# cpuimage/minSDTF

Measured on AMD Instinct MI355X. Metric: 512x512 images/sec (whole node), SD1.5 25-step txt2img, higher is better.
Workload: dtype bf16; 1 GPU; SD1.5 512x512 25-step txt2img, CFG 7.5 + rescale 0.7, batch 1/GPU, UNet+VAE HIP path, random-init weights; global_batch=1, parallelism=batch-shard x1, hipgraph=True, cond_uncond=one fused batch

## Files before the change

### include/minsdtf_hip.h

```cpp
#ifndef MINSDTF_HIP_H
#define MINSDTF_HIP_H

#include <stdint.h>

#ifdef __cplusplus
extern "C" {
#endif

#define MSD_ABI_VERSION 12

#define MSD_OK 0
#define MSD_E_ARG (-1)
#define MSD_E_ALIGN (-2)
#define MSD_E_UNSUPPORTED (-3)
#define MSD_E_WORKSPACE (-4)

typedef void* msd_stream_t;

#if defined(__GNUC__) || defined(__clang__)
#define MSD_API __attribute__((visibility("default")))
#else
#define MSD_API
#endif

MSD_API int msd_abi_version(void);
MSD_API const char* msd_last_error(void);
MSD_API int msd_init(void);
MSD_API int msd_set_option(const char* key, int value);

#define MSD_ACT_NONE 0
#define MSD_ACT_SILU 1
#define MSD_ACT_GEGLU 2
#define MSD_ACT_QUICK_GELU 3

#define MSD_OUT_BF16 0
#define MSD_OUT_F32 1

typedef struct MsdConvGemm {
    const void* a0;
    const void* a1;
    const void* w;
    const float* bias;
    const float* rowvec;
    const int32_t* step_ptr;
    const void* residual;
    void* out;
    void* out1;
    void* out2;
    float* workspace;
    int64_t workspace_floats;
    int32_t batch, h_in, w_in, c0, c1;
    int32_t h_out, w_out;
    int32_t ksize;
    int32_t stride;
    int32_t pad;
    int32_t upsample;
    int32_t N;
    int32_t act;
    int32_t out_dtype;
    int32_t out_ld, res_ld;
    int32_t rv_step_stride, rv_batch_stride;
    int32_t split_mode;
    int32_t ns0, ns1, out1_ld, out2_ld;
    int32_t splitk;
    int32_t tile_n;
    int32_t tile_m;
    int32_t stages;
    const float* ln_in;
    const float* ln_colsum;
    float* ln_out;
    int32_t ln_in_slots;
    int32_t ln_out_slots;
    float ln_eps;
    const void* a2;
    const void* a3;
    int32_t c2, c3;
    int32_t w_layout;
} MsdConvGemm;

MSD_API int msd_conv_gemm_ln_slots(const MsdConvGemm* p);

MSD_API int msd_conv_gemm(const MsdConvGemm* p, msd_stream_t stream);

#define MSD_OUT_U8 2
typedef struct MsdConvDirect {
    const void* in;
    const float* w;
    const float* bias;
    const void* residual;
    void* out;
    int32_t batch, in_batch_mod, h_in, w_in, c_in;
    int32_t h_out, w_out, c_out;
    int32_t ksize, stride, pad;
    int32_t in_dtype;
    int32_t out_dtype;
    int32_t act;
    int32_t act_in;
    float in_scale;
} MsdConvDirect;

MSD_API int msd_conv_direct(const MsdConvDirect* p, msd_stream_t stream);

#define MSD_GN_SYNC_WORDS_PER_SAMPLE 16384
#define MSD_GN_MAX_CHUNKS 1024
typedef struct MsdGroupNorm {
    const void* x0;
    const void* x1;
    const float* gamma;
    const float* beta;
    float* stats;
    float* partials;
    int64_t partials_floats;
    void* out;
    int32_t batch, hw, c0, c1;
    int32_t silu;
    float eps;
    uint32_t* sync;
    int64_t sync_words;
} MsdGroupNorm;

MSD_API int msd_group_norm(const MsdGroupNorm* p, msd_stream_t stream);

MSD_API int msd_layer_norm(const void* x, const float* gamma, const float* beta, void* out, int32_t rows, int32_t c,
                   float eps, msd_stream_t stream);

typedef struct MsdAttention {
    const void* q;
    const void* k;
    const void* vt;
    void* out;
    int32_t batch, heads, head_dim;
    int32_t s, t;
    int32_t q_ld, k_ld, vt_ld, o_ld;
    float scale;
    int32_t causal;
    int32_t q_prescaled;
    float* workspace;
    int64_t workspace_floats;
} MsdAttention;

MSD_API int msd_attention(const MsdAttention* p, msd_stream_t stream);

typedef struct MsdCrossAttnQ {
    const void* x;
    const float* ln_in;
    const void* wq;
    const float* ln_colsum;
    const float* bias;
    const void* k;
    const void* vt;
    void* out;
    int32_t batch, heads, head_dim, s, t;
    int32_t k_ld, vt_ld, o_ld;
    int32_t ln_in_slots;
    float ln_eps;
    int32_t w_layout;
} MsdCrossAttnQ;

MSD_API int msd_cross_attention_q(const MsdCrossAttnQ* p, msd_stream_t stream);

MSD_API int msd_softmax_rows(const float* x, void* out, int64_t rows, int32_t cols, int32_t ld_in, int32_t ld_out, float scale,
                     msd_stream_t stream);

MSD_API int msd_embedding_sum(const int32_t* tokens, const int32_t* positions, const float* tok_table, const float* pos_table,
                      void* out, int32_t rows, int32_t dim, int32_t vocab, int32_t max_len, int32_t* status,
                      msd_stream_t stream);

MSD_API int msd_replicate(const void* src, void* dst, int64_t bytes, int32_t copies, msd_stream_t stream);

MSD_API int msd_memset_zero(void* ptr, int64_t bytes, msd_stream_t stream);

typedef struct MsdCfgStep {
    const float* eps;
    float* latent;
    const float* coef;
    int32_t* step_ptr;
    int32_t batch, n, num_steps;
    float guidance, guidance_rescale;
    int32_t advance;
    const float* inpaint_init;
    const float* inpaint_noise;
    const float* inpaint_mask;
    const float* step_noise;
    const float* noise_coef;
} MsdCfgStep;

MSD_API int msd_cfg_step(const MsdCfgStep* p, msd_stream_t stream);

typedef struct MsdSamplerStep {
    const float* eps;
    float* latent;
    const float* coef;
    int32_t* step_ptr;
    int32_t batch, n, num_steps;
    float guidance, guidance_rescale;
    int32_t advance;
    const float* inpaint_init;
    const float* inpaint_noise;
    const float* inpaint_mask;
    const float* step_noise;
    float* denoised_prev;
} MsdSamplerStep;

MSD_API int msd_sampler_step(const MsdSamplerStep* p, msd_stream_t stream);

typedef struct MsdLoraJob {
    const float* master;
    const float* up;
    const float* down;
    const float* rowscale;
    const float* colscale;
    const int32_t* rowmap;
    void* out;
    void* out_frag;
    float* colsum;
    int32_t n, k, rank, master_ld;
    int32_t layout, out_dtype, ld;
    int32_t out_rows, out_cols, row_off, col_off;
    int32_t first_block;
} MsdLoraJob;

typedef struct MsdLoraMerge {
    const MsdLoraJob* jobs;
    const MsdLoraJob* jobs_dev;
    int32_t num_jobs;
} MsdLoraMerge;

MSD_API int msd_lora_merge(const MsdLoraMerge* p, msd_stream_t stream);

typedef struct MsdResampleRow {
// ... 62 lines not shown
```

### minsdtf_amd/_lib.py

```python
from __future__ import annotations

import atexit
import ctypes as C
import os
import sys
import weakref

LIB_NAME = "libminsdtf_hip.so"
LIB_PATH = os.environ.get("MSD_HIP_LIB") or os.path.join(os.path.dirname(os.path.abspath(__file__)), LIB_NAME)
ABI_VERSION = 12

ACT_NONE, ACT_SILU, ACT_GEGLU, ACT_QUICK_GELU = 0, 1, 2, 3
OUT_BF16, OUT_F32, OUT_U8 = 0, 1, 2


class HipExtensionError(RuntimeError):
    pass


class MsdConvGemm(C.Structure):
    _fields_ = [
        ("a0", C.c_void_p), ("a1", C.c_void_p), ("w", C.c_void_p), ("bias", C.c_void_p), ("rowvec", C.c_void_p),
        ("step_ptr", C.c_void_p), ("residual", C.c_void_p), ("out", C.c_void_p), ("out1", C.c_void_p),
        ("out2", C.c_void_p), ("workspace", C.c_void_p), ("workspace_floats", C.c_int64),
        ("batch", C.c_int32), ("h_in", C.c_int32), ("w_in", C.c_int32), ("c0", C.c_int32), ("c1", C.c_int32),
        ("h_out", C.c_int32), ("w_out", C.c_int32), ("ksize", C.c_int32), ("stride", C.c_int32), ("pad", C.c_int32),
        ("upsample", C.c_int32), ("N", C.c_int32), ("act", C.c_int32), ("out_dtype", C.c_int32),
        ("out_ld", C.c_int32), ("res_ld", C.c_int32), ("rv_step_stride", C.c_int32), ("rv_batch_stride", C.c_int32),
        ("split_mode", C.c_int32), ("ns0", C.c_int32), ("ns1", C.c_int32), ("out1_ld", C.c_int32),
        ("out2_ld", C.c_int32), ("splitk", C.c_int32), ("tile_n", C.c_int32), ("tile_m", C.c_int32), ("stages", C.c_int32),
        ("ln_in", C.c_void_p), ("ln_colsum", C.c_void_p), ("ln_out", C.c_void_p),
        ("ln_in_slots", C.c_int32), ("ln_out_slots", C.c_int32), ("ln_eps", C.c_float),
        ("a2", C.c_void_p), ("a3", C.c_void_p), ("c2", C.c_int32), ("c3", C.c_int32), ("w_layout", C.c_int32),
    ]


class MsdConvDirect(C.Structure):
    _fields_ = [
        ("in_", C.c_void_p), ("w", C.c_void_p), ("bias", C.c_void_p), ("residual", C.c_void_p), ("out", C.c_void_p),
        ("batch", C.c_int32), ("in_batch_mod", C.c_int32), ("h_in", C.c_int32), ("w_in", C.c_int32),
        ("c_in", C.c_int32), ("h_out", C.c_int32), ("w_out", C.c_int32), ("c_out", C.c_int32),
        ("ksize", C.c_int32), ("stride", C.c_int32), ("pad", C.c_int32), ("in_dtype", C.c_int32),
        ("out_dtype", C.c_int32), ("act", C.c_int32), ("act_in", C.c_int32), ("in_scale", C.c_float),
    ]


class MsdGroupNorm(C.Structure):
    _fields_ = [
        ("x0", C.c_void_p), ("x1", C.c_void_p), ("gamma", C.c_void_p), ("beta", C.c_void_p), ("stats", C.c_void_p),
        ("partials", C.c_void_p), ("partials_floats", C.c_int64),
        ("out", C.c_void_p), ("batch", C.c_int32), ("hw", C.c_int32), ("c0", C.c_int32), ("c1", C.c_int32),
        ("silu", C.c_int32), ("eps", C.c_float), ("sync", C.c_void_p), ("sync_words", C.c_int64),
    ]


class MsdCrossAttnQ(C.Structure):
    _fields_ = [
        ("x", C.c_void_p), ("ln_in", C.c_void_p), ("wq", C.c_void_p), ("ln_colsum", C.c_void_p), ("bias", C.c_void_p),
        ("k", C.c_void_p), ("vt", C.c_void_p), ("out", C.c_void_p),
        ("batch", C.c_int32), ("heads", C.c_int32), ("head_dim", C.c_int32), ("s", C.c_int32), ("t", C.c_int32),
        ("k_ld", C.c_int32), ("vt_ld", C.c_int32), ("o_ld", C.c_int32), ("ln_in_slots", C.c_int32), ("ln_eps", C.c_float),
        ("w_layout", C.c_int32),
    ]


class MsdAttention(C.Structure):
    _fields_ = [
        ("q", C.c_void_p), ("k", C.c_void_p), ("vt", C.c_void_p), ("out", C.c_void_p),
        ("batch", C.c_int32), ("heads", C.c_int32), ("head_dim", C.c_int32), ("s", C.c_int32), ("t", C.c_int32),
        ("q_ld", C.c_int32), ("k_ld", C.c_int32), ("vt_ld", C.c_int32), ("o_ld", C.c_int32), ("scale", C.c_float),
        ("causal", C.c_int32), ("q_prescaled", C.c_int32),
        ("workspace", C.c_void_p), ("workspace_floats", C.c_int64),
    ]


class MsdCfgStep(C.Structure):
    _fields_ = [
        ("eps", C.c_void_p), ("latent", C.c_void_p), ("coef", C.c_void_p), ("step_ptr", C.c_void_p),
        ("batch", C.c_int32), ("n", C.c_int32), ("num_steps", C.c_int32), ("guidance", C.c_float),
        ("guidance_rescale", C.c_float), ("advance", C.c_int32),
        ("inpaint_init", C.c_void_p), ("inpaint_noise", C.c_void_p), ("inpaint_mask", C.c_void_p),
        ("step_noise", C.c_void_p), ("noise_coef", C.c_void_p),
    ]


class MsdSamplerStep(C.Structure):
    _fields_ = [
        ("eps", C.c_void_p), ("latent", C.c_void_p), ("coef", C.c_void_p), ("step_ptr", C.c_void_p),
        ("batch", C.c_int32), ("n", C.c_int32), ("num_steps", C.c_int32), ("guidance", C.c_float),
        ("guidance_rescale", C.c_float), ("advance", C.c_int32),
        ("inpaint_init", C.c_void_p), ("inpaint_noise", C.c_void_p), ("inpaint_mask", C.c_void_p),
        ("step_noise", C.c_void_p), ("denoised_prev", C.c_void_p),
    ]


class MsdLoraJob(C.Structure):
    _fields_ = [
        ("master", C.c_void_p), ("up", C.c_void_p), ("down", C.c_void_p), ("rowscale", C.c_void_p), ("colscale", C.c_void_p),
        ("rowmap", C.c_void_p), ("out", C.c_void_p), ("out_frag", C.c_void_p), ("colsum", C.c_void_p),
        ("n", C.c_int32), ("k", C.c_int32), ("rank", C.c_int32), ("master_ld", C.c_int32),
        ("layout", C.c_int32), ("out_dtype", C.c_int32), ("ld", C.c_int32),
        ("out_rows", C.c_int32), ("out_cols", C.c_int32), ("row_off", C.c_int32), ("col_off", C.c_int32),
        ("first_block", C.c_int32),
    ]


class MsdLoraMerge(C.Structure):
    _fields_ = [("jobs", C.c_void_p), ("jobs_dev", C.c_void_p), ("num_jobs", C.c_int32)]


class MsdResampleRow(C.Structure):
    _fields_ = [("idx", C.c_int32 * 4), ("w", C.c_float * 4)]


class MsdLatentResample(C.Structure):
    _fields_ = [
        ("in_", C.c_void_p), ("out", C.c_void_p), ("noise", C.c_void_p), ("wx", C.c_void_p), ("wy", C.c_void_p),
        ("batch", C.c_int32), ("h_in", C.c_int32), ("w_in", C.c_int32), ("h_out", C.c_int32), ("w_out", C.c_int32),
        ("a", C.c_float), ("s", C.c_float),
    ]


TILE_MAX_VIEWS = 64


class MsdTileConsensus(C.Structure):
    _fields_ = [
        ("tiles", C.c_void_p), ("canvas", C.c_void_p), ("ys", C.c_int32 * TILE_MAX_VIEWS), ("xs", C.c_int32 * TILE_MAX_VIEWS),
        ("rows", C.c_int32), ("cols", C.c_int32), ("th", C.c_int32), ("tw", C.c_int32), ("H", C.c_int32), ("W", C.c_int32),
        ("batch", C.c_int32), ("wy", C.c_void_p), ("wx", C.c_void_p), ("mode", C.c_int32),
    ]


REGION_MAX = 16


class MsdRegionCombine(C.Structure):
    _fields_ = [
        ("eps", C.c_void_p), ("w", C.c_void_p), ("out", C.c_void_p),
        ("regions", C.c_int32), ("batch", C.c_int32), ("n", C.c_int32),
    ]


class MsdAttentionIdentity(C.Structure):
    _fields_ = [
        ("vt", C.c_void_p), ("out", C.c_void_p),
        ("batch", C.c_int32), ("channels", C.c_int32), ("s", C.c_int32),
        ("vt_ld", C.c_int32), ("o_ld", C.c_int32),
    ]


LORA_ROWS_PER_BLOCK = 8

SYMBOLS = {
    "msd_abi_version": (C.c_int, []),
    "msd_last_error": (C.c_char_p, []),
    "msd_init": (C.c_int, []),
    "msd_set_option": (C.c_int, [C.c_char_p, C.c_int]),
    "msd_conv_gemm": (C.c_int, [C.POINTER(MsdConvGemm), C.c_void_p]),
    "msd_conv_gemm_ln_slots": (C.c_int, [C.POINTER(MsdConvGemm)]),
    "msd_conv_direct": (C.c_int, [C.POINTER(MsdConvDirect), C.c_void_p]),
    "msd_group_norm": (C.c_int, [C.POINTER(MsdGroupNorm), C.c_void_p]),
    "msd_cross_attention_q": (C.c_int, [C.POINTER(MsdCrossAttnQ), C.c_void_p]),
    "msd_layer_norm": (C.c_int, [C.c_void_p, C.c_void_p, C.c_void_p, C.c_void_p, C.c_int32, C.c_int32, C.c_float,
                                 C.c_void_p]),
    "msd_attention": (C.c_int, [C.POINTER(MsdAttention), C.c_void_p]),
    "msd_softmax_rows": (C.c_int, [C.c_void_p, C.c_void_p, C.c_int64, C.c_int32, C.c_int32, C.c_int32, C.c_float,
                                   C.c_void_p]),
    "msd_memset_zero": (C.c_int, [C.c_void_p, C.c_int64, C.c_void_p]),
    "msd_replicate": (C.c_int, [C.c_void_p, C.c_void_p, C.c_int64, C.c_int32, C.c_void_p]),
    "msd_embedding_sum": (C.c_int, [C.c_void_p, C.c_void_p, C.c_void_p, C.c_void_p, C.c_void_p, C.c_int32, C.c_int32, C.c_int32,
                                    C.c_int32, C.c_void_p, C.c_void_p]),
    "msd_cfg_step": (C.c_int, [C.POINTER(MsdCfgStep), C.c_void_p]),
    "msd_sampler_step": (C.c_int, [C.POINTER(MsdSamplerStep), C.c_void_p]),
    "msd_lora_merge": (C.c_int, [C.POINTER(MsdLoraMerge), C.c_void_p]),
    "msd_latent_resample": (C.c_int, [C.POINTER(MsdLatentResample), C.c_void_p]),
    "msd_tile_consensus": (C.c_int, [C.POINTER(MsdTileConsensus), C.c_void_p]),
    "msd_region_combine": (C.c_int, [C.POINTER(MsdRegionCombine), C.c_void_p]),
    "msd_attention_identity": (C.c_int, [C.POINTER(MsdAttentionIdentity), C.c_void_p]),
    "msd_add_bf16": (C.c_int, [C.c_void_p, C.c_void_p, C.c_void_p, C.c_int64, C.c_void_p]),
    "msd_add_f32_bf16": (C.c_int, [C.c_void_p, C.c_void_p, C.c_void_p, C.c_int64, C.c_void_p]),
    "msd_cast_f32_to_bf16": (C.c_int, [C.c_void_p, C.c_void_p, C.c_int64, C.c_void_p]),
    "msd_cast_bf16_to_f32": (C.c_int, [C.c_void_p, C.c_void_p, C.c_int64, C.c_void_p]),
}

_lib = None
# ... 75 lines not shown
```

### minsdtf_amd/csrc/conv_big.hip

```cpp
#include <type_traits>
#include "conv_common.h"

#ifdef MSD_STAMPS
static __device__ unsigned long long g_bstamps[1024 * 2 * 8];
extern "C" MSD_API int msd_debug_stamps_big(unsigned long long* host_out, int count) {
    return (int)hipMemcpyFromSymbol(host_out, HIP_SYMBOL(g_stamps), sizeof(unsigned long long) * (size_t)count);
}
extern "C" MSD_API int msd_debug_phase_stamps_big(unsigned long long* host_out, int count) {
    return (int)hipMemcpyFromSymbol(host_out, HIP_SYMBOL(g_bstamps), sizeof(unsigned long long) * (size_t)count);
}
#define BSTAMP(i) do { if ((i) < 4) asm volatile("s_memtime %0" : "=s"(bst[i]) : : "memory"); else asm volatile("s_memtime %0\n\ts_waitcnt lgkmcnt(0)" : "=s"(bst[i]) : : "memory"); } while (0)
#define BSTAMP_END()                                                              \
    do {                                                                          \
        asm volatile("s_waitcnt lgkmcnt(0)" ::: "memory");                        \
        _Pragma("unroll") for (int i_ = 0; i_ < 6; ++i_) bsum[i_] += bst[i_ + 1] - bst[i_]; \
        ++bsum[6];                                                                \
    } while (0)
#else
#define BSTAMP(i)
#define BSTAMP_END()
#endif

template <int BM, int BN, int WGM, int WGN, int IH, int JH, int NB>
struct BigGeo {
// ... 266 lines not shown
    const int ca0 = ((g ^ (r >> 1)) << 4), ca1 = (((4 + g) ^ (r >> 1)) << 4);
    const int cw0 = ((g ^ (rw >> 1)) << 4), cw1 = (((4 + g) ^ (rw >> 1)) << 4);
    bf16x8 af[2][IHS], wf0[2][JS0], wf1[2][JS1 > 0 ? JS1 : 1];
    auto load_a = [&](int part, int rb) {
        const char* b = smem + rb * ST_BYTES + aoffs + part * (APR * 128);
#pragma unroll
        for (int ii = 0; ii < IHS; ++ii) {
            af[0][ii] = *reinterpret_cast<const bf16x8*>(b + ii * 2048 + ca0);
            af[1][ii] = *reinterpret_cast<const bf16x8*>(b + ii * 2048 + ca1);
        }
    };
    auto load_w0 = [&](int rb) {
        const char* b = smem + rb * ST_BYTES + woffs0;
#pragma unroll
        for (int jj = 0; jj < JS0; ++jj) {
            wf0[0][jj] = *reinterpret_cast<const bf16x8*>(b + jj * 2048 + cw0);
            wf0[1][jj] = *reinterpret_cast<const bf16x8*>(b + jj * 2048 + cw1);
        }
    };
    auto load_w1 = [&](int rb) {
        const char* b = smem + rb * ST_BYTES + woffs1;
#pragma unroll
        for (int jj = 0; jj < JS1; ++jj) {
            wf1[0][jj] = *reinterpret_cast<const bf16x8*>(b + jj * 2048 + cw0);
            wf1[1][jj] = *reinterpret_cast<const bf16x8*>(b + jj * 2048 + cw1);
        }
    };
    auto mfma_part = [&](auto IP_, auto JP_) {
        constexpr int ip = decltype(IP_)::value, jp = decltype(JP_)::value;
        constexpr int js = jp ? JS1 : JS0;
#pragma unroll
        for (int ks = 0; ks < 2; ++ks)
#pragma unroll
            for (int jj = 0; jj < js; ++jj)
#pragma unroll
                for (int ii = 0; ii < IHS; ++ii) {
                    const int i = ip * IHS + ii, j = jp * JS0 + jj;
                    if constexpr (jp == 0)
                        acc[i / EC][j][i % EC] = __builtin_amdgcn_mfma_f32_16x16x32_bf16(wf0[ks][jj], af[ks][ii], acc[i / EC][j][i % EC], 0, 0, 0);
                    else
                        acc[i / EC][j][i % EC] = __builtin_amdgcn_mfma_f32_16x16x32_bf16(wf1[ks][jj], af[ks][ii], acc[i / EC][j][i % EC], 0, 0, 0);
                }
    };

#ifdef MSD_STAMPS
    unsigned long long bst[7], bsum[7] = {0, 0, 0, 0, 0, 0, 0};
#endif
    int rb = 0, ib = LEADT % NB;
    TileA nt = tile_a(kt_begin + min(LEADT, max(nkt - 1, 0))), ntn = nt;
    prep_phase(std::integral_constant<int, 0>{}, nt);
    auto phase = [&](auto P_, int rem) {
        constexpr int P = decltype(P_)::value;
        BSTAMP(0);
        if constexpr (JH == 2) {
            if constexpr (P == 0) { load_w0(rb); load_a(0, rb); }
            if constexpr (P == 1) load_w1(rb);
            if constexpr (P == 2) load_a(1, rb);
        } else {
            if constexpr (P == 0) load_w0(rb);
            load_a(P, rb);
        }
        __builtin_amdgcn_sched_barrier(0);
        BSTAMP(1);
        if (rem >= LEADT) {
            constexpr int LO = P == 0 ? 0 : Geo::cum(P - 1), HI = Geo::cum(P);
            issue_range(std::integral_constant<int, LO>{}, std::integral_constant<int, HI>{}, nt, ib, std::true_type{});
        }
        BSTAMP(2);
        if constexpr (P + 1 < PH) {
            if constexpr (Geo::need(P + 1) > Geo::need(P)) {
                constexpr int base = G - 1 - Geo::need(P + 1);
                if (rem >= LEADT) wait_vmcnt<(base + (LEADT - 1) * G + Geo::cum(P) < 63 ? base + (LEADT - 1) * G + Geo::cum(P) : 63)>();
                else big_wait(base + rem * G);
            }
        } else {
            constexpr int base = G - 1 - Geo::need(0);
            if (rem >= LEADT) wait_vmcnt<(base + (LEADT - 1) * G < 63 ? base + (LEADT - 1) * G : 63)>();
            else if (rem >= 1) big_wait(base + (rem - 1) * G);
        }
        BSTAMP(3);
        __builtin_amdgcn_s_barrier();
        BSTAMP(4);
        __builtin_amdgcn_sched_barrier(0);
        __builtin_amdgcn_s_setprio(1);
        if constexpr (P + 1 < PH) prep_phase(std::integral_constant<int, P + 1>{}, nt);
        else prep_phase(std::integral_constant<int, 0>{}, ntn);
        if constexpr (JH == 2) {
            if constexpr (P == 0) mfma_part(std::integral_constant<int, 0>{}, std::integral_constant<int, 0>{});
            if constexpr (P == 1) mfma_part(std::integral_constant<int, 0>{}, std::integral_constant<int, 1>{});
            if constexpr (P == 2) mfma_part(std::integral_constant<int, 1>{}, std::integral_constant<int, 1>{});
            if constexpr (P == 3) mfma_part(std::integral_constant<int, 1>{}, std::integral_constant<int, 0>{});
        } else {
            mfma_part(std::integral_constant<int, P>{}, std::integral_constant<int, 0>{});
        }
#pragma unroll
        for (int q = 0; q < 24; ++q) {
            __builtin_amdgcn_sched_group_barrier(0x008, 1, 0);
            __builtin_amdgcn_sched_group_barrier(0x006, 2, 0);
        }
#pragma unroll
        for (int q = 0; q < (PA > 0 ? PA : 1); ++q) asm volatile("" : "+v"(pa[q]));
        __builtin_amdgcn_s_setprio(0);
        __builtin_amdgcn_sched_barrier(0);
        BSTAMP(5);
        __builtin_amdgcn_s_barrier();
        BSTAMP(6);
        BSTAMP_END();
    };
    for (int t = 0; t < nkt; ++t) {
        const int rem = nkt - 1 - t;
        if (rem > LEADT) ntn = tile_a(kt_begin + t + 1 + LEADT);
#ifdef MSD_STAMPS
        if (t == 0) MSD_STAMP(2);
        if (t == (nkt >> 1)) MSD_STAMP(5);
#endif
        phase(std::integral_constant<int, 0>{}, rem);
        phase(std::integral_constant<int, 1>{}, rem);
        if constexpr (PH == 4) {
            phase(std::integral_constant<int, 2>{}, rem);
            phase(std::integral_constant<int, 3>{}, rem);
        }
        if (++rb == NB) rb = 0;
        if (++ib == NB) ib = 0;
        nt = ntn;
    }
    if (grp == 0) __builtin_amdgcn_s_barrier();
    MSD_STAMP(3);
#ifdef MSD_STAMPS
    if ((wave & 3) == 0 && lane == 0) {
        unsigned long long* dst = g_bstamps + ((size_t)(blockIdx.x & 1023) * 2 + grp) * 8;
#pragma unroll
        for (int i = 0; i < 7; ++i) dst[i] = bsum[i];
    }
#endif

    auto epilogue_chunk = [&](auto H_) {
        constexpr int h = decltype(H_)::value;
        int mrow[EC];
#pragma unroll
        for (int i = 0; i < EC; ++i) mrow[i] = m0 + wm * WMT + (h * EC + i) * 16;
        cg_epilogue<EC, NJ, false, DENSE>(p, acc[h], mrow, n0 + wn * WNT, r, g, reinterpret_cast<float*>(smem), wn, WGN, wm * WMT + h * EC * 16, BM, tile_n);
    };
    epilogue_chunk(std::integral_constant<int, 0>{});
    if constexpr (EH > 1) epilogue_chunk(std::integral_constant<int, 1>{});
    if constexpr (EH > 2) epilogue_chunk(std::integral_constant<int, 2>{});
    if constexpr (EH > 3) epilogue_chunk(std::integral_constant<int, 3>{});
    static_assert(EH <= 4 && MI % EC == 0, "epilogue chunks");
#ifdef MSD_STAMPS
    asm volatile("s_waitcnt vmcnt(0)" ::: "memory");
    MSD_STAMP(4);
#endif
}

template <int BN, int WGM, int WGN, int NBW>
__global__ __launch_bounds__(512) void conv_bighalo_kernel(CG_HOT_PARAMS, const CGArgs p) {
    CG_HOT_UNPACK;
    constexpr int BM = 256, HW_ = 18, HROWS = 18 * 18, HPAD = 336;
    static_assert(WGM * WGN == 8 && BN % 32 == 0 && BN % (WGN * 16) == 0, "tile");
    constexpr int WMT = BM / WGM, WNT = BN / WGN, MI = WMT / 16, NJ = WNT / 16, IHS = MI / 2;
    static_assert(MI % 2 == 0 && MI * WGM == 16, "a wave owns MI image rows of the 16 x 16 tile, read in two parts");
    constexpr int H_BYTES = HPAD * 128, W_BYTES = BN * 128;
    constexpr int WRF = BN / 64, WRH = (BN % 64) / 32, WR = WRF + WRH, W0 = (WR + 1) / 2;
    constexpr int LEAD = NBW - 1;
    static_assert(LEAD >= 1 && LEAD <= 3, "weight steps in flight (the halo RAW rule needs <= 3)");
    static_assert(2 * H_BYTES + NBW * W_BYTES <= 160 * 1024, "LDS");
    constexpr int NWAIT = LEAD + WR * (LEAD - 1);
    extern __shared__ __attribute__((aligned(16))) char smem[];
    const uint32_t lds0 = (uint32_t)(size_t)(__attribute__((address_space(3))) char*)smem;

    const int tid = threadIdx.x, lane = tid & 63;
    const int wave = __builtin_amdgcn_readfirstlane(tid >> 6);
    const int wm = wave / WGN, wn = wave - wm * WGN;
    const int grp = wave >> 2;
    const int r = lane & 15, g = lane >> 4;
    MSD_STAMP(0);
    const int ups = p.upsample ? 1 : 0;
    const int Hl = p.h_in << ups, Wl = p.w_in << ups;
    const int tiles_x = Wl >> 4, tps = tiles_x * (Hl >> 4);
    const int tile = xcd_remap(blockIdx.x, hot_tiles_m * hot_tiles_n);
    const int tdiv = hot_m_fast ? hot_tiles_m : hot_tiles_n;
    const int tq = udiv_magic(tile, tdiv, hot_mg_tdiv), tr = tile - tq * tdiv;
    const int tile_n = hot_m_fast ? tq : tr;
    const int tmi = hot_m_fast ? tr : tq;
    const int b = udiv_magic(tmi, tps, p.mg_tps);
    const int trem = tmi - b * tps;
    const int tyi = udiv_magic(trem, tiles_x, p.mg_tx);
    const int ty0 = tyi * 16, tx0 = (trem - tyi * tiles_x) * 16;
    const int n0 = tile_n * BN;
    const int c_begin = blockIdx.y * hot_nk_per;
    const int nch = min(p.nkc, c_begin + hot_nk_per) - c_begin;
    const int nkt = nch * 9;

    const int cpos = lane & 7, lr8 = lane >> 3;
    const char* zero = reinterpret_cast<const char*>(g_zero_page) + cpos * 16;
    int hpix[6];
#pragma unroll
    for (int k = 0; k < 6; ++k) {
        const int hrow = k < 5 ? 64 * k + 8 * wave + lr8 : 320 + 2 * wave + (lr8 & 1);
        const int hy = (hrow * 3641) >> 16, hx = hrow - hy * HW_;
        const int iy = ty0 + hy - 1, ix = tx0 + hx - 1;
        const bool ok = hrow < HROWS && (unsigned)iy < (unsigned)Hl && (unsigned)ix < (unsigned)Wl;
        const int pix = (b * p.h_in + (min(max(iy, 0), Hl - 1) >> ups)) * p.w_in + (min(max(ix, 0), Wl - 1) >> ups);
        hpix[k] = ok ? pix : -1;
    }
    const uint32_t hsrc = (uint32_t)((cpos ^ ((4 * wave + (lane >> 4)) & 7)) * 16);
    const uint32_t hsrc5 = (uint32_t)((cpos ^ (wave & 7)) * 16);
    uint32_t woff[WR];
#pragma unroll
    for (int k = 0; k < WR; ++k) {
        const int q = 64 * k + (k >= WRF ? 4 : 8) * wave + lr8;
        woff[k] = (uint32_t)min(n0 + q, hot_N - 1) * hot_w_rs + (uint32_t)((cpos ^ ((q >> 1) & 7)) * 16);
    }
    const uint32_t ldsH_wave = lds0 + (uint32_t)(wave * 8) * 128u;
    const uint32_t ldsH5_wave = lds0 + (uint32_t)(320 + wave * 2) * 128u;
    const uint32_t ldsW_wave = lds0 + 2u * H_BYTES + (uint32_t)(wave * 8) * 128u;
    const uint32_t ldsWh_wave = lds0 + 2u * H_BYTES + (uint32_t)(wave * 4) * 128u;

    struct ChunkA { uint64_t sb; uint32_t csrc2; };
    auto chunk_a = [&](int c) {
        const int ch = c * 64;
        const bool first = ch < hot_c0;
        ChunkA t;
        t.sb = (uint64_t)(first ? hot_a0 : hot_a1) + (uint64_t)(uint32_t)((first ? ch : ch - hot_c0) * 2);
        t.csrc2 = (uint32_t)(first ? hot_c0 : hot_c1) * 2u;
        return t;
    };
    auto halo_addr = [&](auto K_, const ChunkA& t, bool live) -> uint64_t {
        constexpr int k = decltype(K_)::value;
        const uint32_t off = __umul24((uint32_t)hpix[k], t.csrc2) + (k < 5 ? hsrc : hsrc5);
        const uint32_t m32 = (uint32_t)(~hpix[k] >> 31) & (live ? 0xFFFFFFFFu : 0u);
        const uint64_t m64 = ((uint64_t)m32 << 32) | m32;
        return ((t.sb + off) & m64) | ((uint64_t)zero & ~m64);
    };
    auto fire_halo = [&](auto K_, uint64_t a, int hb) {
        constexpr int k = decltype(K_)::value;
        const uint32_t boff = (uint32_t)hb * (uint32_t)H_BYTES;
        if constexpr (k < 5) dma16(reinterpret_cast<const void*>(a), ldsH_wave + boff + (uint32_t)k * 8192u);
        else if constexpr (k == 5) dma16m(reinterpret_cast<const void*>(a), ldsH5_wave + boff, 0xFFFFull);
        else dma16(zero, lds0 + boff + 328u * 128u);
    };
    auto issue_w = [&](auto LO_, auto HI_, uint32_t koff, int ib) {
        constexpr int LO = decltype(LO_)::value, HI = decltype(HI_)::value;
        const uint32_t boff = (uint32_t)ib * (uint32_t)W_BYTES;
#pragma unroll
        for (int k = LO; k < HI; ++k) {
            const char* wb = reinterpret_cast<const char*>(hot_w) + koff;
            if (k < WRF) dma16s(wb, woff[k], ldsW_wave + boff + (uint32_t)k * 8192u);
            else dma16sm(wb, woff[k], ldsWh_wave + boff + (uint32_t)k * 8192u, 0xFFFFFFFFull);
        }
    };
    auto w_koff = [&](int c, int tap) { return (uint32_t)(tap * p.nkc + c) * hot_w_ks; };

    constexpr int EC = 2, EH = MI / EC;
    f32x4 acc[EH][NJ][EC];
#pragma unroll
    for (int h = 0; h < EH; ++h)
#pragma unroll
        for (int j = 0; j < NJ; ++j)
#pragma unroll
            for (int i = 0; i < EC; ++i) acc[h][j][i] = (f32x4){0.f, 0.f, 0.f, 0.f};

    {
        const ChunkA t = chunk_a(c_begin);
        fire_halo(std::integral_constant<int, 0>{}, halo_addr(std::integral_constant<int, 0>{}, t, true), 0);
        fire_halo(std::integral_constant<int, 1>{}, halo_addr(std::integral_constant<int, 1>{}, t, true), 0);
        fire_halo(std::integral_constant<int, 2>{}, halo_addr(std::integral_constant<int, 2>{}, t, true), 0);
        fire_halo(std::integral_constant<int, 3>{}, halo_addr(std::integral_constant<int, 3>{}, t, true), 0);
        fire_halo(std::integral_constant<int, 4>{}, halo_addr(std::integral_constant<int, 4>{}, t, true), 0);
        fire_halo(std::integral_constant<int, 5>{}, halo_addr(std::integral_constant<int, 5>{}, t, true), 0);
#pragma unroll
        for (int tt = 0; tt < LEAD; ++tt) {
            issue_w(std::integral_constant<int, 0>{}, std::integral_constant<int, WR>{}, w_koff(c_begin, tt), tt);
            fire_halo(std::integral_constant<int, 6>{}, 0, 1);
        }
    }
    MSD_STAMP(1);
    wait_vmcnt<1 + (LEAD - 1) * (WR + 1)>();
    __builtin_amdgcn_s_barrier();
    if (grp == 1) __builtin_amdgcn_s_barrier();

    const int rw = cg_wrow(r);
    const int woffs = 2 * H_BYTES + (wn * WNT + rw) * 128;
    const int cw0 = ((g ^ (rw >> 1)) << 4), cw1 = (((4 + g) ^ (rw >> 1)) << 4);
    bf16x8 af[2][IHS], wf[2][NJ];
    int fa[IHS];
    auto prep_frag = [&](int part, int ky, int kx, int hb) {
#pragma unroll
        for (int ii = 0; ii < IHS; ++ii) {
            const int hr = (wm * MI + part * IHS + ii + ky) * HW_ + kx + r;
            fa[ii] = hb * H_BYTES + hr * 128 + ((g ^ ((hr >> 1) & 7)) << 4);
        }
    };
    auto load_a = [&]() {
#pragma unroll
        for (int ii = 0; ii < IHS; ++ii) {
            af[0][ii] = *reinterpret_cast<const bf16x8*>(smem + fa[ii]);
            af[1][ii] = *reinterpret_cast<const bf16x8*>(smem + (fa[ii] ^ 64));
        }
    };
    auto load_w = [&](int rb) {
        const char* bw = smem + rb * W_BYTES + woffs;
#pragma unroll
        for (int jj = 0; jj < NJ; ++jj) {
            wf[0][jj] = *reinterpret_cast<const bf16x8*>(bw + jj * 2048 + cw0);
            wf[1][jj] = *reinterpret_cast<const bf16x8*>(bw + jj * 2048 + cw1);
        }
    };
    auto mfma_part = [&](auto IP_) {
        constexpr int ip = decltype(IP_)::value;
#pragma unroll
        for (int ks = 0; ks < 2; ++ks)
#pragma unroll
            for (int jj = 0; jj < NJ; ++jj)
#pragma unroll
                for (int ii = 0; ii < IHS; ++ii) {
                    const int i = ip * IHS + ii;
                    acc[i / EC][jj][i % EC] = __builtin_amdgcn_mfma_f32_16x16x32_bf16(wf[ks][jj], af[ks][ii], acc[i / EC][jj][i % EC], 0, 0, 0);
                }
    };
    auto mfma_slot_open = [&]() {
        __builtin_amdgcn_s_barrier();
        __builtin_amdgcn_sched_barrier(0);
        __builtin_amdgcn_s_setprio(1);
    };
    auto mfma_slot_close = [&]() {
#pragma unroll
        for (int q = 0; q < 24; ++q) {
            __builtin_amdgcn_sched_group_barrier(0x008, 1, 0);
            __builtin_amdgcn_sched_group_barrier(0x006, 2, 0);
        }
#pragma unroll
        for (int ii = 0; ii < IHS; ++ii) asm volatile("" : "+v"(fa[ii]));
        __builtin_amdgcn_s_setprio(0);
        __builtin_amdgcn_sched_barrier(0);
        __builtin_amdgcn_s_barrier();
    };

    int rb = 0, ib = LEAD % NBW;
    prep_frag(0, 0, 0, 0);
    uint64_t ph = 0;
    ChunkA nx = chunk_a(c_begin);
    for (int c = 0; c < nch; ++c) {
        const int hb = c & 1;
        const bool has_next = c + 1 < nch;
        if (has_next) nx = chunk_a(c_begin + c + 1);
#ifdef MSD_STAMPS
        if (c == 0) MSD_STAMP(2);
        if (c == (nch >> 1)) MSD_STAMP(5);
#endif
        auto step = [&](auto TAP_) {
            constexpr int TAP = decltype(TAP_)::value;
            constexpr int ky = TAP / 3, kx = TAP - ky * 3;
            constexpr int TAPW = (TAP + LEAD) % 9, CW = (TAP + LEAD) / 9;
            constexpr int TAPN = (TAP + 1) % 9;
            const int rem = nkt - 1 - (c * 9 + TAP);
            const uint32_t koff = w_koff(c_begin + c + CW, TAPW);
            load_w(rb);
            load_a();
            __builtin_amdgcn_sched_barrier(0);
            if (rem >= LEAD) issue_w(std::integral_constant<int, 0>{}, std::integral_constant<int, W0>{}, koff, ib);
            mfma_slot_open();
            prep_frag(1, ky, kx, hb);
            if constexpr (TAP < 6) ph = halo_addr(std::integral_constant<int, TAP>{}, nx, has_next);
            mfma_part(std::integral_constant<int, 0>{});
            if constexpr (TAP < 6) asm volatile("" : "+v"(ph));
            mfma_slot_close();
            load_a();
            __builtin_amdgcn_sched_barrier(0);
            if (rem >= LEAD) issue_w(std::integral_constant<int, W0>{}, std::integral_constant<int, WR>{}, koff, ib);
            if constexpr (TAP < 6) fire_halo(std::integral_constant<int, TAP>{}, ph, hb ^ 1);
            else fire_halo(std::integral_constant<int, 6>{}, 0, hb ^ 1);
            if (rem >= LEAD) wait_vmcnt<NWAIT>();
            else if (rem >= 1) big_wait(LEAD + WR * max(0, min(LEAD - 1, rem - 1)));
            mfma_slot_open();
            prep_frag(0, TAPN / 3, TAPN % 3, TAP == 8 ? hb ^ 1 : hb);
            mfma_part(std::integral_constant<int, 1>{});
            mfma_slot_close();
            if (++rb == NBW) rb = 0;
            if (++ib == NBW) ib = 0;
        };
        step(std::integral_constant<int, 0>{}); step(std::integral_constant<int, 1>{}); step(std::integral_constant<int, 2>{});
        step(std::integral_constant<int, 3>{}); step(std::integral_constant<int, 4>{}); step(std::integral_constant<int, 5>{});
        step(std::integral_constant<int, 6>{}); step(std::integral_constant<int, 7>{}); step(std::integral_constant<int, 8>{});
    }
    if (grp == 0) __builtin_amdgcn_s_barrier();
    wait_vmcnt<0>();

    const int nxc = p.nk - p.nk_main;
    if (nxc > 0) {
        const int eps = (nxc + p.nslices - 1) / p.nslices;
        const int e0 = min(nxc, (int)blockIdx.y * eps), e1 = min(nxc, e0 + eps);
        const int cx3 = p.K - p.nk_main * 64 - p.c2;
        auto issue_extra = [&](int e, int slot) {
            const int ce = e * 64;
            const bool first = ce < p.c2;
            const uint64_t sb = (uint64_t)(first ? p.a2 : p.a3) + (uint64_t)(uint32_t)((first ? ce : ce - p.c2) * 2);
            const uint32_t cs2 = (uint32_t)(first ? p.c2 : cx3) * 2u;
            const uint32_t base = __builtin_amdgcn_readfirstlane(ldsH_wave + (uint32_t)slot * (uint32_t)H_BYTES);
#pragma unroll
            for (int k = 0; k < 4; ++k) {
                const int q = 64 * k + 8 * wave + lr8;
                const int pix = (b * Hl + ty0 + (q >> 4)) * Wl + tx0 + (q & 15);
                dma16(reinterpret_cast<const void*>(sb + (__umul24((uint32_t)pix, cs2) + hsrc)), base + (uint32_t)k * 8192u);
            }
            issue_w(std::integral_constant<int, 0>{}, std::integral_constant<int, WR>{}, (uint32_t)(p.nk_main + e) * hot_w_ks, slot);
        };
        auto prep_xfrag = [&](int part, int slot) {
#pragma unroll
            for (int ii = 0; ii < IHS; ++ii) {
                const int q = (wm * MI + part * IHS + ii) * 16 + r;
                fa[ii] = slot * H_BYTES + q * 128 + ((g ^ ((q >> 1) & 7)) << 4);
            }
        };
        int slot = 0;
        if (e0 < e1) issue_extra(e0, 0);
        for (int e = e0; e < e1; ++e) {
            wait_vmcnt<0>();
            __builtin_amdgcn_s_barrier();
            if (e + 1 < e1) issue_extra(e + 1, slot ^ 1);
            load_w(slot);
            prep_xfrag(0, slot);
            load_a();
            mfma_part(std::integral_constant<int, 0>{});
            prep_xfrag(1, slot);
            load_a();
            mfma_part(std::integral_constant<int, 1>{});
            slot ^= 1;
        }
    }
    MSD_STAMP(3);

    auto epilogue_chunk = [&](auto H_) {
        constexpr int h = decltype(H_)::value;
        int mrow[EC];
#pragma unroll
        for (int i = 0; i < EC; ++i) mrow[i] = (b * Hl + ty0 + wm * MI + h * EC + i) * Wl + tx0;
        cg_epilogue<EC, NJ, true, false>(p, acc[h], mrow, n0 + wn * WNT, r, g);
    };
    epilogue_chunk(std::integral_constant<int, 0>{});
    if constexpr (EH > 1) epilogue_chunk(std::integral_constant<int, 1>{});
    if constexpr (EH > 2) epilogue_chunk(std::integral_constant<int, 2>{});
    if constexpr (EH > 3) epilogue_chunk(std::integral_constant<int, 3>{});
    static_assert(EH <= 4, "epilogue chunks");
#ifdef MSD_STAMPS
    asm volatile("s_waitcnt vmcnt(0)" ::: "memory");
    MSD_STAMP(4);
#endif
}

#ifndef MSD_BIG_CFGS
#define MSD_BIG_CFGS(X)          \
    X(256, 256, 2, 4, 2, 2, 2, 0) \
    X(256, 160, 4, 2, 2, 2, 3, 0) \
    X(256, 160, 4, 2, 2, 1, 3, 1) \
    X(256, 160, 4, 2, 2, 2, 2, 2) \
    X(256, 128, 4, 2, 2, 1, 3, 0) \
    X(256, 128, 4, 2, 2, 2, 3, 1) \
    X(128, 256, 2, 4, 2, 1, 3, 0) \
    X(128, 256, 2, 4, 2, 2, 3, 1)
#endif

constexpr int big_lds(int bm, int bn, int nb) { return nb * (bm + bn) * 128; }

#ifndef MSD_BIGHALO_CFGS
#define MSD_BIGHALO_CFGS(X) \
    X(160, 4, 2, 3, 0)      \
    X(128, 4, 2, 3, 0)      \
    X(128, 4, 2, 4, 1)
#endif
constexpr int bighalo_lds(int bn, int nbw) { return 2 * 336 * 128 + nbw * bn * 128; }

static bool g_big_attr_done = false;
static int msd_conv_big_init() {
    if (g_big_attr_done) return MSD_OK;
    hipError_t e = hipSuccess;
#define X(bm, bn, wgm, wgn, ih, jh, nb, code)                                                                                 \
    if (e == hipSuccess)                                                                                                      \
        e = hipFuncSetAttribute(reinterpret_cast<const void*>(&conv_big_kernel<bm, bn, wgm, wgn, ih, jh, nb, 0>),             \
                                hipFuncAttributeMaxDynamicSharedMemorySize, big_lds(bm, bn, nb));                             \
    if (e == hipSuccess)                                                                                                      \
        e = hipFuncSetAttribute(reinterpret_cast<const void*>(&conv_big_kernel<bm, bn, wgm, wgn, ih, jh, nb, 1>),             \
                                hipFuncAttributeMaxDynamicSharedMemorySize, big_lds(bm, bn, nb));                             \
    if (e == hipSuccess)                                                                                                      \
        e = hipFuncSetAttribute(reinterpret_cast<const void*>(&conv_big_kernel<bm, bn, wgm, wgn, ih, jh, nb, 2>),             \
                                hipFuncAttributeMaxDynamicSharedMemorySize, big_lds(bm, bn, nb));
    MSD_BIG_CFGS(X)
#undef X
#define X(bn, wgm, wgn, nbw, code)                                                                                            \
    if (e == hipSuccess)                                                                                                      \
        e = hipFuncSetAttribute(reinterpret_cast<const void*>(&conv_bighalo_kernel<bn, wgm, wgn, nbw>),                       \
                                hipFuncAttributeMaxDynamicSharedMemorySize, bighalo_lds(bn, nbw));
    MSD_BIGHALO_CFGS(X)
#undef X
    if (e != hipSuccess) MSD_FAIL((int)e, "hipFuncSetAttribute(conv_big): %s", hipGetErrorString(e));
    g_big_attr_done = true;
    return MSD_OK;
}

int msd_conv_big_nj(const CGForm& f) {
#define X(bm_, bn_, wgm, wgn, ih, jh, nb, code_) if (f.rows == bm_ && f.cols == bn_ && f.code == code_) return bn_ / wgn / 16;
    MSD_BIG_CFGS(X)
#undef X
    return 0;
}

int msd_conv_big_launch(const CGArgs& a, const CGForm& f, int slices, bool dense, hipStream_t stream) {
    int rc = msd_conv_big_init();
    if (rc) return rc;
    const dim3 grid(a.tiles_m * a.tiles_n, slices);
#define X(bm_, bn_, wgm, wgn, ih, jh, nb, code_)                                                                              \
    if (f.rows == bm_ && f.cols == bn_ && f.code == code_) {                                                                  \
        if (dense)                                                                                                            \
            hipLaunchKernelGGL((conv_big_kernel<bm_, bn_, wgm, wgn, ih, jh, nb, 1>), grid, dim3(512),                         \
                               big_lds(bm_, bn_, nb), stream, CG_HOT_ARGS(a), a);                                             \
        else if (a.upsample)                                                                                                  \
            hipLaunchKernelGGL((conv_big_kernel<bm_, bn_, wgm, wgn, ih, jh, nb, 2>), grid, dim3(512),                         \
                               big_lds(bm_, bn_, nb), stream, CG_HOT_ARGS(a), a);                                             \
        else                                                                                                                  \
            hipLaunchKernelGGL((conv_big_kernel<bm_, bn_, wgm, wgn, ih, jh, nb, 0>), grid, dim3(512),                         \
                               big_lds(bm_, bn_, nb), stream, CG_HOT_ARGS(a), a);                                             \
        return MSD_OK;                                                                                                        \
    }
    MSD_BIG_CFGS(X)
#undef X
    MSD_FAIL(MSD_E_UNSUPPORTED, "conv_big: no %d x %d configuration with code %d", f.rows, f.cols, f.code);
}

int msd_conv_bighalo_nj(const CGForm& f) {
#define X(bn_, wgm, wgn, nbw, code_) if (f.cols == bn_ && f.code == code_) return bn_ / wgn / 16;
    MSD_BIGHALO_CFGS(X)
#undef X
    return 0;
}

int msd_conv_bighalo_launch(const CGArgs& a, const CGForm& f, int slices, hipStream_t stream) {
    int rc = msd_conv_big_init();
    if (rc) return rc;
    const dim3 grid(a.tiles_m * a.tiles_n, slices);
#define X(bn_, wgm, wgn, nbw, code_)                                                                                          \
    if (f.cols == bn_ && f.code == code_) {                                                                                   \
        hipLaunchKernelGGL((conv_bighalo_kernel<bn_, wgm, wgn, nbw>), grid, dim3(512), bighalo_lds(bn_, nbw), stream,         \
                           CG_HOT_ARGS(a), a);                                                                                \
        return MSD_OK;                                                                                                        \
    }
    MSD_BIGHALO_CFGS(X)
#undef X
    MSD_FAIL(MSD_E_UNSUPPORTED, "conv_big: no halo-image configuration 256 x %d with code %d", f.cols, f.code);
}
```

### minsdtf_amd/csrc/conv_common.h

```cpp
#pragma once
#include "common.h"

struct CGArgs {
    const bf16_t* a0; const bf16_t* a1; const bf16_t* w;
    const float* bias; const float* rowvec; const int32_t* step_ptr;
    const bf16_t* residual; void* out; bf16_t* out1; bf16_t* out2; float* ws;
    int batch, h_in, w_in, c0, c1, h_out, w_out, ksize, stride, pad, upsample;
    int M, N, K, hw_out, nkc, nk, nk_per, tiles_n;
    int nslices;
    int tiles_m, m_fast;
    int act, out_f32, out_ld, res_ld, rv_step_stride, rv_batch_stride;
    int vec16;
    int split_mode, ns0, ns1, out1_ld, out2_ld;
    uint32_t mg_tdiv, mg_hw, mg_w, mg_tps, mg_tx, mg_nkc;
    const bf16_t* a2; const bf16_t* a3; int c2, nk_main;
    const float* ln_in; const float* ln_colsum; float* ln_out;
    int ln_in_slots, ln_out_slots;
    float ln_eps, ln_inv_k;
    int kmajor;
    uint32_t w_rs, w_ks;
};
#include "conv_form.h"

#define CG_HOT_PARAMS const bf16_t* hot_a0, const bf16_t* hot_w, const bf16_t* hot_a1, int hot_M, int hot_N, uint32_t hot_pk_c, uint32_t hot_pk_tiles, \
                      uint32_t hot_pk_nk, uint32_t hot_mg_tdiv, uint32_t hot_w_rs, uint32_t hot_w_ks
#define CG_HOT_ARGS(a) (a).a0, (a).w, (a).a1, (a).M, (a).N, ((uint32_t)(a).c0 | ((uint32_t)(a).c1 << 16)),                           \
                       ((uint32_t)(a).tiles_m | ((uint32_t)(a).tiles_n << 23) | ((uint32_t)((a).m_fast ? 1u : 0u) << 31)),          \
                       ((uint32_t)(a).nk_per | ((uint32_t)(a).nk << 16)), (a).mg_tdiv, (a).w_rs, (a).w_ks
#define CG_HOT_UNPACK                                                                                                          \
    const int hot_c0 = (int)(hot_pk_c & 0xFFFFu), hot_c1 = (int)(hot_pk_c >> 16);                                             \
    const int hot_tiles_m = (int)(hot_pk_tiles & 0x7FFFFFu), hot_tiles_n = (int)((hot_pk_tiles >> 23) & 0xFFu);                \
    const int hot_m_fast = (int)(hot_pk_tiles >> 31);                                                                          \
    const int hot_nk_per = (int)(hot_pk_nk & 0xFFFFu), hot_nk = (int)(hot_pk_nk >> 16);                                        \
    (void)hot_c1; (void)hot_a1; (void)hot_w_rs; (void)hot_w_ks; (void)hot_nk
static inline bool cg_hot_ok(const CGArgs& a) {
    return a.c0 >= 0 && a.c0 < 65536 && a.c1 >= 0 && a.c1 < 65536 && a.tiles_m > 0 && a.tiles_m < (1 << 23) && a.tiles_n > 0 && a.tiles_n < 256 &&
           a.nk_per > 0 && a.nk_per < 65536 && a.nk > 0 && a.nk < 65536;
}

static __device__ __attribute__((aligned(128))) uint32_t g_zero_page[32];


#ifdef MSD_STAMPS
static __device__ unsigned long long g_stamps[16 * 8192];
#define MSD_STAMP(i)                                                                                             \
    do {                                                                                                         \
        if (threadIdx.x == 0) g_stamps[(((size_t)blockIdx.y * gridDim.x + blockIdx.x) & 8191) * 16 + (i)] = wall_clock64(); \
    } while (0)
#define MSD_STAMP_DRAIN() asm volatile("s_waitcnt vmcnt(0)" ::: "memory")
#else
#define MSD_STAMP(i)
#define MSD_STAMP_DRAIN()
#endif

__device__ __forceinline__ void cg_store4(const CGArgs& p, int m, int b, int n, int step, float v[4]) {
    if (p.bias) {
        const float4 bv = *reinterpret_cast<const float4*>(p.bias + n);
        v[0] += bv.x; v[1] += bv.y; v[2] += bv.z; v[3] += bv.w;
    }
    if (p.rowvec) {
        const float4 rv = *reinterpret_cast<const float4*>(
            p.rowvec + (size_t)step * p.rv_step_stride + (size_t)b * p.rv_batch_stride + n);
        v[0] += rv.x; v[1] += rv.y; v[2] += rv.z; v[3] += rv.w;
    }
    if (p.act == MSD_ACT_SILU) {
#pragma unroll
        for (int e = 0; e < 4; ++e) v[e] = silu_f(v[e]);
    } else if (p.act == MSD_ACT_QUICK_GELU) {
#pragma unroll
        for (int e = 0; e < 4; ++e) v[e] = v[e] * fast_rcp(1.0f + __expf(-1.702f * v[e]));
    }
    if (p.split_mode == 0) {
        if (p.residual) {
            const uint2 rr = *reinterpret_cast<const uint2*>(p.residual + (size_t)m * p.res_ld + n);
            v[0] += bf_lo(rr.x); v[1] += bf_hi(rr.x); v[2] += bf_lo(rr.y); v[3] += bf_hi(rr.y);
        }
        if (p.out_f32) {
            *reinterpret_cast<float4*>(reinterpret_cast<float*>(p.out) + (size_t)m * p.out_ld + n) =
                make_float4(v[0], v[1], v[2], v[3]);
        } else {
            uint2 o; o.x = pack_bf2(v[0], v[1]); o.y = pack_bf2(v[2], v[3]);
            *reinterpret_cast<uint2*>(reinterpret_cast<bf16_t*>(p.out) + (size_t)m * p.out_ld + n) = o;
        }
    } else {
        uint2 o; o.x = pack_bf2(v[0], v[1]); o.y = pack_bf2(v[2], v[3]);
        if (n < p.ns0) {
            *reinterpret_cast<uint2*>(reinterpret_cast<bf16_t*>(p.out) + (size_t)m * p.out_ld + n) = o;
        } else if (n < p.ns0 + p.ns1) {
            *reinterpret_cast<uint2*>(p.out1 + (size_t)m * p.out1_ld + (n - p.ns0)) = o;
        } else {
            const int nv = p.N - p.ns0 - p.ns1;
            const int nn = n - p.ns0 - p.ns1;
            const int s = m - b * p.hw_out;
            bf16_t* dst = p.out2 + ((size_t)b * nv + nn) * p.out2_ld + s;
            dst[0] = (bf16_t)(o.x & 0xFFFF);
            dst[(size_t)p.out2_ld] = (bf16_t)(o.x >> 16);
            dst[(size_t)2 * p.out2_ld] = (bf16_t)(o.y & 0xFFFF);
            dst[(size_t)3 * p.out2_ld] = (bf16_t)(o.y >> 16);
        }
    }
}

__device__ __forceinline__ void cg_store4_pre(const CGArgs& p, int m, int b, int n, float v[4], float4 bv, bool has_b, float4 rv, bool has_rv,
                                              uint2 rr, bool has_r) {
    if (has_b) { v[0] += bv.x; v[1] += bv.y; v[2] += bv.z; v[3] += bv.w; }
    if (has_rv) { v[0] += rv.x; v[1] += rv.y; v[2] += rv.z; v[3] += rv.w; }
    if (p.act == MSD_ACT_SILU) {
#pragma unroll
        for (int e = 0; e < 4; ++e) v[e] = silu_f(v[e]);
    } else if (p.act == MSD_ACT_QUICK_GELU) {
#pragma unroll
        for (int e = 0; e < 4; ++e) v[e] = v[e] * fast_rcp(1.0f + __expf(-1.702f * v[e]));
    }
    if (p.split_mode == 0) {
        if (has_r) { v[0] += bf_lo(rr.x); v[1] += bf_hi(rr.x); v[2] += bf_lo(rr.y); v[3] += bf_hi(rr.y); }
        if (p.out_f32) {
            *reinterpret_cast<float4*>(reinterpret_cast<float*>(p.out) + (size_t)m * p.out_ld + n) = make_float4(v[0], v[1], v[2], v[3]);
        } else {
            uint2 o; o.x = pack_bf2(v[0], v[1]); o.y = pack_bf2(v[2], v[3]);
            *reinterpret_cast<uint2*>(reinterpret_cast<bf16_t*>(p.out) + (size_t)m * p.out_ld + n) = o;
        }
        return;
    }
    uint2 o; o.x = pack_bf2(v[0], v[1]); o.y = pack_bf2(v[2], v[3]);
    if (n < p.ns0) {
        *reinterpret_cast<uint2*>(reinterpret_cast<bf16_t*>(p.out) + (size_t)m * p.out_ld + n) = o;
    } else if (n < p.ns0 + p.ns1) {
        *reinterpret_cast<uint2*>(p.out1 + (size_t)m * p.out1_ld + (n - p.ns0)) = o;
    } else {
        const int nv = p.N - p.ns0 - p.ns1;
        const int nn = n - p.ns0 - p.ns1;
        const int sidx = m - b * p.hw_out;
        bf16_t* dst = p.out2 + ((size_t)b * nv + nn) * p.out2_ld + sidx;
        dst[0] = (bf16_t)(o.x & 0xFFFF);
        dst[(size_t)p.out2_ld] = (bf16_t)(o.x >> 16);
        dst[(size_t)2 * p.out2_ld] = (bf16_t)(o.y & 0xFFFF);
        dst[(size_t)3 * p.out2_ld] = (bf16_t)(o.y >> 16);
    }
}

constexpr int LN_MAX_SLOTS = 20;
__device__ __forceinline__ int cg_wrow(int r) { return (r & 3) | ((r & 4) << 1) | ((r & 8) >> 1); }
__device__ __forceinline__ int cg_col(int g) { return ((g & 1) << 3) | ((g & 2) << 1); }
template <int MI, int NJ, bool UB = false, bool DF = true>
__device__ __forceinline__ void cg_epilogue(const CGArgs& p, f32x4 (&acc)[NJ][MI], const int (&mrow)[MI], int nbase, int r, int g,
                                            float* lnred = nullptr, int wn = 0, int wgn = 1, int row0 = 0, int bm = 0, int tile_n = 0) {
    const int cgo = cg_col(g);
    if (p.nslices > 1) {
        float* ws = p.ws + (size_t)blockIdx.y * p.M * p.N;
#pragma unroll
        for (int i = 0; i < MI; ++i) {
            const int m = mrow[i] + r;
            if (m >= p.M) continue;
#pragma unroll
            for (int j = 0; j < NJ; ++j) {
                const int n = nbase + j * 16 + cgo;
                if (n >= p.N) continue;
                *reinterpret_cast<float4*>(ws + (size_t)m * p.N + n) =
                    make_float4(acc[j][i][0], acc[j][i][1], acc[j][i][2], acc[j][i][3]);
            }
        }
        return;
    }
    const int step = p.step_ptr ? *p.step_ptr : 0;
    constexpr int MP = MI / 2;
    const bool v16 = (MI % 2 == 0) && p.vec16;
    const int cg8 = (g & 1) << 3;
    int msw[MP > 0 ? MP : 1];
#pragma unroll
    for (int ip = 0; ip < MP; ++ip) msw[ip] = (g < 2 ? mrow[2 * ip] : mrow[2 * ip + 1]) + r;
    auto swap8 = [&](const float (&a)[4], const float (&b)[4], float (&v)[8]) {
#pragma unroll
        for (int e = 0; e < 4; ++e) {
// ... 345 lines not shown
```

### minsdtf_amd/csrc/conv_form.h

```cpp
#pragma once

enum CGFamily {
    CG_TILE,
    CG_HALO,
    CG_ROWPANEL,
    CG_WREG,
    CG_BIG,
    CG_BIGHALO,
    CG_NONE
};
struct CGForm {
    CGFamily family;
    bool valid;
    int rows;
    int cols;
    int code;
    bool chunk_major;
    int variant;
    int th;
};
static inline CGForm cg_decode_form(int tile_m, int tile_n, int stages) {
    const int walk = stages >= 20 ? 2 : stages >= 10 ? 1 : 0;
    CGForm f = {CG_TILE, tile_m >= 0 && tile_m < 6000, tile_m, tile_n, stages, false, 0, 0};
    if (tile_m >= 6000) f.family = CG_NONE;
    else if (tile_m < 1000) f.variant = walk;
    else if (tile_m >= 5000) {
        f.family = walk == 2 ? CG_BIGHALO : CG_BIG;
        f.rows = tile_m - 5000; f.code = stages - 10 * walk; f.chunk_major = walk > 0;
    } else if (tile_m >= 3000) {
        f.family = tile_m >= 4000 ? CG_WREG : CG_ROWPANEL;
        f.rows = tile_m % 1000;
    } else if (tile_m >= 1000) {
        f.family = CG_HALO;
        f.rows = tile_m % 1000; f.th = f.rows / 16; f.variant = tile_m >= 2000 ? 1 : 0; f.chunk_major = true;
    }
    return f;
}
static inline bool cg_is_big(const CGForm& f) { return f.family == CG_BIG || f.family == CG_BIGHALO; }

int msd_conv_halo_launch(const CGArgs& a, const CGForm& f, int slices, hipStream_t stream);
bool msd_conv_rowpanel_eligible(const CGArgs& a, int rows, int wg_cols);
int msd_conv_rowpanel_launch(CGArgs a, int rows, int wg_cols, hipStream_t stream);
int msd_conv_wreg_nj(const CGForm& f);
int msd_conv_wreg_launch(const CGArgs& a, const CGForm& f, int slices, bool dense, hipStream_t stream);
int msd_conv_big_nj(const CGForm& f);
int msd_conv_big_launch(const CGArgs& a, const CGForm& f, int slices, bool dense, hipStream_t stream);
int msd_conv_bighalo_nj(const CGForm& f);
int msd_conv_bighalo_launch(const CGArgs& a, const CGForm& f, int slices, hipStream_t stream);
```

### minsdtf_amd/csrc/conv_gemm.hip

```cpp
#include "conv_common.h"

#ifdef MSD_STAMPS
extern "C" MSD_API int msd_debug_stamps(unsigned long long* host_out, int count) {
    return (int)hipMemcpyFromSymbol(host_out, HIP_SYMBOL(g_stamps), sizeof(unsigned long long) * (size_t)count);
}
#endif

template <int BM, int BN, int WGM, int WGN, int S, bool DENSE>
__global__ __launch_bounds__(WGM * WGN * 64) void conv_gemm_dma_kernel(CG_HOT_PARAMS, const CGArgs p) {
    CG_HOT_UNPACK;
    constexpr int NW = WGM * WGN;
    constexpr int NT = NW * 64;
    constexpr int WMT = BM / WGM, WNT = BN / WGN;
    constexpr int MI = WMT / 16, NJ = WNT / 16;
    constexpr int RPP = NT / 8;
    constexpr int BNP = (BN + RPP - 1) / RPP * RPP;
    constexpr int AR = BM * 8 / NT, BR = BNP * 8 / NT;
    static_assert(AR >= 1 && BR >= 1 && (BM * 8) % NT == 0 && WMT % 16 == 0 && WNT % 16 == 0, "tile config");
    constexpr int L = AR + BR;
    constexpr int A_BYTES = BM * 128, B_BYTES = BNP * 128, ST_BYTES = A_BYTES + B_BYTES;
    extern __shared__ __attribute__((aligned(16))) char smem[];
    const uint32_t lds0 = (uint32_t)(size_t)(__attribute__((address_space(3))) char*)smem;

    const int tid = threadIdx.x, lane = tid & 63;
// ... 284 lines not shown
    if (run.family == CG_HALO && run.th == 16 && run.cols != 80) run.cols = 128;
    if (run.family == CG_TILE && run.rows == 0) run.rows = 128;
    if (run.family == CG_TILE && run.variant == 1 && q->act == MSD_ACT_GEGLU) run.code = 0;
    return run;
}

static void cg_set_tiles(CGArgs& a, int tiles_m, int cols, int tps = 0, int tx = 0) {
    a.tiles_m = tiles_m;
    a.tiles_n = (a.N + cols - 1) / cols;
    a.m_fast = (a.N > a.M) ? 1 : 0;
    a.mg_tdiv = udiv_magic_of(a.m_fast ? a.tiles_m : a.tiles_n);
    a.mg_tps = tps ? udiv_magic_of(tps) : 0;
    a.mg_tx = tx ? udiv_magic_of(tx) : 0;
}
static int cg_dense_form(const MsdConvGemm* q, const CGArgs& a, bool tile, bool* dense) {
    const bool needs_dense = q->ln_in || q->act == MSD_ACT_GEGLU || q->split_mode;
    bool d = !q->rowvec && !q->a2 && q->ksize == 1 && q->stride == 1 && !q->upsample && q->h_out == q->h_in && q->w_out == q->w_in;
    if (tile)
        d = d && (g_conv_dense || needs_dense) && (long long)a.M * (q->c0 > q->c1 ? q->c0 : q->c1) * 2 < (1ll << 32) - 4096 &&
            (long long)a.N * a.K * 2 < (1ll << 32) - 4096;
    if (needs_dense && !d)
        MSD_FAIL(MSD_E_UNSUPPORTED, "conv_gemm: the LayerNorm fold, GEGLU and the q|k|v^T split run on the 1x1 / Dense form only%s",
                 tile ? " (ksize 1, stride 1, no upsampling, no rowvec, no shortcut operand)" : "");
    *dense = d;
    return MSD_OK;
}
static int cg_hot_check(const CGArgs& a) {
    if (!cg_hot_ok(a)) MSD_FAIL(MSD_E_UNSUPPORTED, "conv_gemm: tile / K-tile / channel counts beyond the packed launch arguments (K tiles, channels < 65536; row tiles < 2^23; column tiles < 256)");
    return MSD_OK;
}
static int cg_launched(int rc, const CGArgs& a, int slices, hipStream_t stream) {
    if (rc) return rc;
    MSD_CHECK_LAUNCH();
    if (slices > 1) {
        launch_finalize(a, slices, stream);
        MSD_CHECK_LAUNCH();
    }
    return MSD_OK;
}

static int cg_tile_cfg(const CGForm& f) {
    int cfg = -1;
#define X(id, bm, bn, wgm, wgn, st, code_) if (f.rows == bm && f.cols == bn && (cfg < 0 || f.code == code_)) cfg = id;
    MSD_TILE_CFGS(X)
#undef X
    return cfg;
}
static void cg_tile_launch(int cfg, const CGArgs& a, bool dense, int slices, hipStream_t stream) {
    const dim3 grid(a.tiles_m * a.tiles_n, slices);
    switch (cfg) {
#define X(id, bm_, bn_, wgm, wgn, st, code)                                                                             \
    case id:                                                                                                            \
        if (dense)                                                                                                      \
            hipLaunchKernelGGL((conv_gemm_dma_kernel<bm_, bn_, wgm, wgn, st, true>), grid, dim3(wgm * wgn * 64),        \
                               cfg_lds(bm_, bn_, wgm * wgn * 64, st), stream, CG_HOT_ARGS(a), a);                       \
        else                                                                                                            \
            hipLaunchKernelGGL((conv_gemm_dma_kernel<bm_, bn_, wgm, wgn, st, false>), grid, dim3(wgm * wgn * 64),       \
                               cfg_lds(bm_, bn_, wgm * wgn * 64, st), stream, CG_HOT_ARGS(a), a);                       \
        break;
        MSD_TILE_CFGS(X)
#undef X
    }
}


extern "C" int msd_conv_gemm(const MsdConvGemm* q, msd_stream_t stream_) {
    hipStream_t stream = (hipStream_t)stream_;
    if (!q) MSD_FAIL(MSD_E_ARG, "conv_gemm: null params");
    if (!q->a0 || !q->w) MSD_FAIL(MSD_E_ARG, "conv_gemm: null a0/w");
    if (!q->out && !(q->split_mode == 1 && q->ns0 == 0)) MSD_FAIL(MSD_E_ARG, "conv_gemm: null out");
    if (q->batch <= 0 || q->h_in <= 0 || q->w_in <= 0 || q->h_out <= 0 || q->w_out <= 0)
        MSD_FAIL(MSD_E_ARG, "conv_gemm: non-positive dims");
    if (q->c0 <= 0 || (q->c0 % 64) || q->c1 < 0 || (q->c1 % 64) || (q->c1 > 0 && !q->a1))
        MSD_FAIL(MSD_E_ARG, "conv_gemm: channel counts must be positive multiples of 64 (c0=%d c1=%d)", q->c0, q->c1);
    if (!((q->ksize == 1 && q->pad == 0) || (q->ksize == 3 && (q->pad == 0 || q->pad == 1))))
        MSD_FAIL(MSD_E_UNSUPPORTED, "conv_gemm: ksize/pad %d/%d", q->ksize, q->pad);
    if (q->stride != 1 && q->stride != 2) MSD_FAIL(MSD_E_UNSUPPORTED, "conv_gemm: stride %d", q->stride);
    {
        const int hl = q->upsample ? 2 * q->h_in : q->h_in, wl = q->upsample ? 2 * q->w_in : q->w_in;
        auto dim_ok = [&](int in, int out) {
            for (int e = 0; e <= (q->ksize == 3 ? 1 : 0); ++e) {
                const int span = in + q->pad + e - q->ksize;
                if (span >= 0 && span / q->stride + 1 == out) return true;
            }
            return false;
        };
        if (!dim_ok(hl, q->h_out) || !dim_ok(wl, q->w_out))
            MSD_FAIL(MSD_E_ARG, "conv_gemm: output dims %dx%d do not match the geometry (in %dx%d, k%d s%d pad %d)", q->h_out,
                     q->w_out, hl, wl, q->ksize, q->stride, q->pad);
    }
    if (q->N <= 0 || (q->N % 4)) MSD_FAIL(MSD_E_ARG, "conv_gemm: N=%d must be a positive multiple of 4", q->N);
    if (!msd_aligned16(q->a0) || !msd_aligned16(q->a1) || !msd_aligned16(q->w) || !msd_aligned16(q->out) ||
        !msd_aligned16(q->bias) || !msd_aligned16(q->rowvec) || !msd_aligned16(q->residual) ||
        !msd_aligned16(q->workspace) || !msd_aligned16(q->out1) || !msd_aligned16(q->out2))
        MSD_FAIL(MSD_E_ALIGN, "conv_gemm: pointers must be 16-byte aligned");
    if ((q->out_ld % 4) || (q->residual && (q->res_ld % 4)) || (q->rv_step_stride % 4) || (q->rv_batch_stride % 4))
        MSD_FAIL(MSD_E_ALIGN, "conv_gemm: leading dimensions must be multiples of 4");
    if (q->act < 0 || q->act > 3) MSD_FAIL(MSD_E_ARG, "conv_gemm: act");
    if (q->act == MSD_ACT_GEGLU && ((q->N % 32) || q->out_dtype != MSD_OUT_BF16 || q->split_mode || q->rowvec))
        MSD_FAIL(MSD_E_UNSUPPORTED, "conv_gemm: GEGLU needs N%%32==0, bf16 out, plain mode");
    if (q->split_mode) {
        if (q->split_mode != 1 || (q->ns0 % 4) || (q->ns1 % 4) || q->ns0 < 0 || q->ns1 < 0 || q->ns0 + q->ns1 > q->N ||
            q->out_dtype != MSD_OUT_BF16 || q->residual || q->act == MSD_ACT_GEGLU)
            MSD_FAIL(MSD_E_ARG, "conv_gemm: bad split mode arguments");
        if ((q->ns0 > 0 && (q->out_ld % 4)) || (q->ns1 > 0 && (!q->out1 || (q->out1_ld % 4))) ||
            (q->ns0 + q->ns1 < q->N && (!q->out2 || q->out2_ld < q->h_out * q->w_out)))
            MSD_FAIL(MSD_E_ARG, "conv_gemm: split outputs");
    }
    int rc = msd_conv_gemm_init();
    if (rc) return rc;

    CGArgs a;
    a.a0 = (const bf16_t*)q->a0; a.a1 = (const bf16_t*)q->a1; a.w = (const bf16_t*)q->w;
    a.bias = q->bias; a.rowvec = q->rowvec; a.step_ptr = q->step_ptr;
    a.residual = (const bf16_t*)q->residual; a.out = q->out; a.out1 = (bf16_t*)q->out1; a.out2 = (bf16_t*)q->out2;
    a.ws = q->workspace;
    a.batch = q->batch; a.h_in = q->h_in; a.w_in = q->w_in; a.c0 = q->c0; a.c1 = q->c1;
    a.h_out = q->h_out; a.w_out = q->w_out; a.ksize = q->ksize; a.stride = q->stride; a.pad = q->pad;
    a.upsample = q->upsample ? 1 : 0;
    a.hw_out = q->h_out * q->w_out;
    a.mg_hw = udiv_magic_of(a.hw_out);
    a.mg_w = udiv_magic_of(a.w_out);
    const long long M = (long long)q->batch * a.hw_out;
    if (M > (1ll << 30)) MSD_FAIL(MSD_E_ARG, "conv_gemm: M too large");
    a.M = (int)M; a.N = q->N;
    const int cin = q->c0 + q->c1;
    a.K = q->ksize * q->ksize * cin;
    a.nkc = cin / 64;
    a.mg_nkc = udiv_magic_of(a.nkc);
    if ((long long)q->batch * q->h_in * q->w_in * (q->c0 > q->c1 ? q->c0 : q->c1) * 2 >= (1ll << 32) - 4096 ||
        (long long)q->N * q->ksize * q->ksize * cin * 2 >= (1ll << 32) - 4096)
        MSD_FAIL(MSD_E_UNSUPPORTED, "conv_gemm: an operand of 4 GB or more");
    a.nk = q->ksize * q->ksize * a.nkc;
    a.act = q->act; a.out_f32 = (q->out_dtype == MSD_OUT_F32);
    a.out_ld = q->out_ld; a.res_ld = q->res_ld;
    a.rv_step_stride = q->rv_step_stride; a.rv_batch_stride = q->rv_batch_stride;
    a.split_mode = q->split_mode; a.ns0 = q->ns0; a.ns1 = q->ns1; a.out1_ld = q->out1_ld; a.out2_ld = q->out2_ld;
    a.vec16 = (q->N % 8 == 0) && (q->out_ld % 8 == 0) && (!q->residual || q->res_ld % 8 == 0) &&
              (!q->split_mode || ((q->ns0 % 16) == 0 && (q->ns1 % 16) == 0 && (q->ns1 == 0 || q->out1_ld % 8 == 0)));

    a.a2 = (const bf16_t*)q->a2; a.a3 = (const bf16_t*)q->a3; a.c2 = q->c2; a.nk_main = a.nk;
    if (q->a2) {
        if (q->c2 <= 0 || (q->c2 % 64) || q->c3 < 0 || (q->c3 % 64) || (q->c3 > 0 && !q->a3) || q->stride != 1 || q->upsample ||
            q->h_out != q->h_in || q->w_out != q->w_in || !msd_aligned16(q->a2) || !msd_aligned16(q->a3))
            MSD_FAIL(MSD_E_ARG, "conv_gemm: shortcut operand needs stride 1, a same-size output and channel counts that are multiples of 64");
        if ((long long)a.M * (q->c2 > q->c3 ? q->c2 : q->c3) * 2 >= (1ll << 32) - 4096) MSD_FAIL(MSD_E_UNSUPPORTED, "conv_gemm: an operand of 4 GB or more");
        a.K += q->c2 + q->c3;
        a.nk += (q->c2 + q->c3) / 64;
    } else if (q->c2 || q->c3 || q->a3) {
        MSD_FAIL(MSD_E_ARG, "conv_gemm: c2 / c3 / a3 without a2");
    }
    if ((long long)a.N * a.K * 2 >= (1ll << 32) - 4096) MSD_FAIL(MSD_E_UNSUPPORTED, "conv_gemm: an operand of 4 GB or more");
    if (q->w_layout < 0 || q->w_layout > 2) MSD_FAIL(MSD_E_ARG, "conv_gemm: w_layout %d", q->w_layout);
    const CGForm f = cg_decode_form(q->tile_m, q->tile_n, q->stages);
    if (!f.valid) MSD_FAIL(MSD_E_ARG, "conv_gemm: tile_m %d names no kernel form", q->tile_m);
    const bool wreg = f.family == CG_WREG, big = cg_is_big(f), bighalo = f.family == CG_BIGHALO;
    if (big) {
        if (f.chunk_major && (q->ksize != 3 || (q->a2 && !bighalo)))
            MSD_FAIL(MSD_E_UNSUPPORTED, "conv_gemm: the chunk-major walk of the big-tile form is for 3x3 convs (with a shortcut operand: on the staged-halo variant only)");
        if (bighalo) {
            if (f.rows != 256 || !msd_conv_bighalo_nj(f))
                MSD_FAIL(MSD_E_UNSUPPORTED, "conv_gemm: no halo-image big-tile configuration %d x %d code %d", f.rows, f.cols, f.code);
            const int up = q->upsample ? 2 : 1;
            if (q->stride != 1 || q->pad != 1 || q->h_out != up * q->h_in || q->w_out != up * q->w_in || (q->h_out % 16) || (q->w_out % 16))
                MSD_FAIL(MSD_E_UNSUPPORTED, "conv_gemm: the halo-image big-tile form runs 3x3 / stride 1 / pad 1 convs on output images of whole 16 x 16-pixel tiles (%d x %d)", q->h_out, q->w_out);
        } else if (!msd_conv_big_nj(f))
            MSD_FAIL(MSD_E_UNSUPPORTED, "conv_gemm: no big-tile configuration %d x %d code %d", f.rows, f.cols, f.code);
        if (q->ln_out) MSD_FAIL(MSD_E_UNSUPPORTED, "conv_gemm: the big-tile form has no LayerNorm-producer epilogue (ln_out)");
        if ((long long)q->batch * q->h_in * q->w_in >= (1ll << 24) || (long long)(q->c0 > q->c1 ? q->c0 : q->c1) * 2 >= (1ll << 24))
            MSD_FAIL(MSD_E_UNSUPPORTED, "conv_gemm: big-tile form needs fewer than 2^24 input pixels");
        if ((long long)q->batch * q->h_in * q->w_in * (q->c0 > q->c1 ? q->c0 : q->c1) * 2 >= (1ll << 32) - 4096)
            MSD_FAIL(MSD_E_UNSUPPORTED, "conv_gemm: big-tile form needs input tensors under 4 GB");
        if (q->a2 && ((long long)q->batch * q->h_out * q->w_out >= (1ll << 24) || (long long)(q->c2 > q->c3 ? q->c2 : q->c3) * 2 >= (1ll << 24)))
            MSD_FAIL(MSD_E_UNSUPPORTED, "conv_gemm: big-tile form needs fewer than 2^24 output pixels / shortcut row bytes");
    }
    if (wreg != (q->w_layout == 2))
        MSD_FAIL(MSD_E_ARG, "conv_gemm: tile_m %d with w_layout %d (the fragment-major weight image, w_layout 2, is read by the wreg form, tile_m 4000 + rows, and by nothing else)",
                 q->tile_m, q->w_layout);
    if (wreg && ((q->N % 16) || !msd_conv_wreg_nj(f)))
        MSD_FAIL(MSD_E_UNSUPPORTED, "conv_gemm: no wreg configuration %d x %d stages %d (N %% 16 must be 0: N = %d)", f.rows, f.cols, f.code, q->N);
    a.w_rs = q->w_layout ? 128u : (uint32_t)a.K * 2u;
    a.w_ks = q->w_layout ? (uint32_t)a.N * 128u : 128u;
    a.ln_in = q->ln_in; a.ln_colsum = q->ln_colsum; a.ln_out = q->ln_out;
    a.ln_in_slots = q->ln_in_slots; a.ln_out_slots = q->ln_out_slots; a.ln_eps = q->ln_eps;
    a.ln_inv_k = 1.0f / (float)a.K;
    if (q->ln_in) {
        if (!q->ln_colsum || q->ln_in_slots < 1 || q->ln_in_slots > LN_MAX_SLOTS || q->ksize != 1 || !(q->ln_eps > 0.f))
            MSD_FAIL(MSD_E_ARG, "conv_gemm: LayerNorm fold needs ln_colsum, 1 <= ln_in_slots <= %d, ksize 1, ln_eps > 0", LN_MAX_SLOTS);
        if (!msd_aligned16(q->ln_colsum) || (((uintptr_t)q->ln_in) & 7u)) MSD_FAIL(MSD_E_ALIGN, "conv_gemm: ln_in / ln_colsum alignment");
    }
    if (q->ln_out) {
        if (q->split_mode || q->out_dtype != MSD_OUT_BF16 || q->act != MSD_ACT_NONE || q->ksize != 1 || f.family == CG_HALO || big ||
            (((uintptr_t)q->ln_out) & 7u))
            MSD_FAIL(MSD_E_ARG, "conv_gemm: ln_out needs a plain 1x1 launch with a bf16 output and no activation");
        if (q->ln_out_slots != msd_conv_gemm_ln_slots(q))
            MSD_FAIL(MSD_E_ARG, "conv_gemm: ln_out_slots=%d, this launch writes %d partials per row", q->ln_out_slots,
                     msd_conv_gemm_ln_slots(q));
    }

    const int splitk = q->splitk < 1 ? 1 : q->splitk;
    if ((q->ln_in || q->ln_out) && splitk > 1) MSD_FAIL(MSD_E_UNSUPPORTED, "conv_gemm: the LayerNorm fold is plain-K only (splitk=%d)", splitk);
    const CGForm run = cg_resolve_form(f, q, a, splitk);
    const int slices = a.nslices;
    if (slices > 1) {
        if (q->split_mode || q->act == MSD_ACT_GEGLU) MSD_FAIL(MSD_E_UNSUPPORTED, "conv_gemm: split-K needs plain mode");
        if ((long long)a.M * a.N / 4 >= (1ll << 31)) MSD_FAIL(MSD_E_UNSUPPORTED, "conv_gemm: split-K output too large");
        if (!q->workspace || q->workspace_floats < (long long)slices * a.M * a.N)
            MSD_FAIL(MSD_E_WORKSPACE, "conv_gemm: split-K workspace too small (%lld < %lld floats)",
                     (long long)q->workspace_floats, (long long)slices * a.M * a.N);
    }
    bool dense = false;
    switch (run.family) {
    case CG_HALO: {
        const int ty = a.h_in / run.th, tx = a.w_in / 16;
        cg_set_tiles(a, a.batch * ty * tx, run.cols, ty * tx, tx);
        rc = msd_conv_halo_launch(a, run, slices, stream);
        break;
    }
    case CG_ROWPANEL:
        rc = msd_conv_rowpanel_launch(a, run.rows, run.cols, stream);
        break;
    case CG_WREG:
    case CG_BIG:
        if (q->act == MSD_ACT_GEGLU && ((wreg ? msd_conv_wreg_nj(run) : msd_conv_big_nj(run)) % 2))
            MSD_FAIL(MSD_E_UNSUPPORTED, "conv_gemm: GEGLU needs x | gate fragment pairs per wave");
        cg_set_tiles(a, (a.M + run.rows - 1) / run.rows, run.cols);
        if ((rc = cg_dense_form(q, a, false, &dense)) || (rc = cg_hot_check(a))) return rc;
        rc = wreg ? msd_conv_wreg_launch(a, run, slices, dense, stream) : msd_conv_big_launch(a, run, slices, dense, stream);
        break;
    case CG_BIGHALO: {
        const int ty = a.h_out / 16, tx = a.w_out / 16;
        cg_set_tiles(a, a.batch * ty * tx, run.cols, ty * tx, tx);
        if ((rc = cg_hot_check(a))) return rc;
        rc = msd_conv_bighalo_launch(a, run, slices, stream);
        break;
    }
    default: {
        const int cfg = cg_tile_cfg(run);
        if (cfg < 0)
            MSD_FAIL(MSD_E_ARG, "conv_gemm: unsupported tile %dx%d (have 128x128 128x64 64x64 64x128 256x128)", run.rows, run.cols);
        cg_set_tiles(a, (a.M + run.rows - 1) / run.rows, run.cols);
        if ((rc = cg_hot_check(a)) || (rc = cg_dense_form(q, a, true, &dense))) return rc;
        cg_tile_launch(cfg, a, dense, slices, stream);
    }
    }
    return cg_launched(rc, a, slices, stream);
}
```

### minsdtf_amd/engine.py

```python
from __future__ import annotations

import os
import weakref
from dataclasses import dataclass
from typing import Callable, Dict, List, Optional, Sequence, Tuple

import numpy as np
import torch

from . import _lib, ops, packing, tuning
from . import weights as wtab

EPS = 1e-5


class Arena:

    ALIGN = 256

    def __init__(self):
        self.free_list: List[Tuple[int, int]] = []
        self.top = 0
        self.base: Optional[int] = None
        self.storage: Optional[torch.Tensor] = None
# ... 125 lines not shown
        self.recs.append(lambda: fn(**kw))

    @property
    def ws(self):
        return _Lazy(lambda: self._ws_buf.ptr if self._ws_buf is not None else None)

    @property
    def gn_partials(self):
        return _Lazy(lambda: self._gn_part_buf.ptr)

    @property
    def gn_sync(self):
        return _Lazy(lambda: self._gn_sync_buf.ptr)

    def gn_stats_slot(self, batch: int):
        slot = self.gn_slots
        self.gn_slots += 1
        self.gn_batch = max(self.gn_batch, batch)
        return _Lazy(lambda: self._stats_buf.ptr + slot * self.gn_batch * 64 * 4)

    def finalize(self) -> None:
        if self.ws_floats:
            self._ws_buf = self._alloc_tail(self.ws_floats * 4)
        if self.gn_slots:
            self._stats_buf = self._alloc_tail(self.gn_slots * self.gn_batch * 64 * 4)
            self._gn_part_buf = self._alloc_tail(self.gn_batch * ops.GN_MAX_CHUNKS * 64 * 4)
            self._gn_sync_buf = self._alloc_tail(self.gn_batch * ops.GN_SYNC_WORDS_PER_SAMPLE * 4)
        self.arena.materialize(self.device, self.high_water)
        if self._gn_sync_buf is not None and torch.device(self.device).type == "cuda":
            _gn_sync_plans.add(self)
        self.calls = [r() for r in self.recs]
        self.recs = []

    def run(self, stream: int) -> None:
        self.run_range(stream, 0, None)

    def run_range(self, stream: int, lo: int, hi: Optional[int] = None) -> None:
        if not TRACE:
            for c in self.calls[lo:hi]:
                c(stream)
            return
        cur = None
        for c in self.calls[lo:hi]:
            blk = _block_of(c.name)
            if blk != cur:
                if cur is not None:
                    torch.cuda.nvtx.range_pop()
                torch.cuda.nvtx.range_push(blk)
                cur = blk
            c(stream)
        if cur is not None:
            torch.cuda.nvtx.range_pop()


TRACE = os.environ.get("MSD_TRACE", "0") == "1"

_gn_sync_plans: "weakref.WeakSet[Plan]" = weakref.WeakSet()
GN_GIVE_UP_WORD = 8
GN_EPOCH = 0


def retire_stale(cache: dict) -> int:
    stale = [k for k in cache if k[-1] != GN_EPOCH]
    for k in stale:
        owner = cache.pop(k)
        rel = getattr(owner, "release_graphs", None)
        if rel is not None:
            rel()
    if stale:
        import gc

        gc.collect()
    return len(stale)


def gn_sync_flags(device=None) -> Optional[torch.Tensor]:
    plans = _gn_plans_on(device)
    if not plans:
        return None
    words = [p._gn_sync_buf.tensor(torch.int32, (GN_GIVE_UP_WORD + 1,))[GN_GIVE_UP_WORD:] for p in plans]
    return torch.cat(words)


def _gn_plans_on(device):
    return [p for p in _gn_sync_plans if device is None or torch.device(p.device) == torch.device(device)]


def check_gn_sync(flags=None, device=None, group_wide: bool = False) -> None:
    global GN_EPOCH
    if flags is None:
        dev_flags = gn_sync_flags(device)
        flags = None if dev_flags is None else dev_flags.cpu()
    worst = 0 if flags is None else int(flags.max())
    from . import dist as mdist

    if group_wide and mdist.collectives_on():
        import torch.distributed as tdist

        backend_cuda = tdist.get_backend() == "nccl"
        t = torch.tensor([worst], dtype=torch.int32, device=torch.device("cuda", torch.cuda.current_device()) if backend_cuda else "cpu")
        tdist.all_reduce(t, op=tdist.ReduceOp.MAX)
        worst = int(t.item())
    if worst == 0:
        return
    for p in _gn_plans_on(device):
        p._gn_sync_buf.tensor(torch.int32, (GN_GIVE_UP_WORD + 1,))[GN_GIVE_UP_WORD].zero_()
    GN_EPOCH += 1
    _lib.check(_lib.load().msd_set_option(b"gn_cluster", 0), "gn_cluster")
    raise _lib.HipExtensionError(
        "msd_group_norm: a workgroup of the cluster GroupNorm gave up waiting for its group's partial moments (sync word [8] "
        "set, on this rank or another one of the process group): this job's result is wrong and has been discarded.  The cluster "
        "kernel is now off for this process (msd_set_option('gn_cluster', 0): the one-workgroup-per-group path has no exchange) "
        "and the launch plans will be recorded again: retry the call")


def _block_of(call_name: str) -> str:
    parts = call_name.split(".")
    n = 4 if parts[0] in ("down_blocks", "up_blocks") else 3 if parts[0] == "mid_block" else 2 if parts[0] in ("decoder", "encoder") else 1
    return ".".join(parts[:n])


class _Lazy:

    def __init__(self, fn):
        self.fn = fn

    @property
    def ptr(self):
        return self.fn()


def _tile_n(N: int) -> int:
    return 128 if (N % 128 == 0 or N > 1024) else 64


def pick_splitk(M: int, N: int, nk: int) -> int:
    tiles = ((M + 127) // 128) * ((N + _tile_n(N) - 1) // _tile_n(N))
    if tiles >= 160 or nk < 32:
        return 1
    s = min((256 + tiles - 1) // tiles, nk // 8, 16)
    return max(1, s)


LN_FOLD = True
FF_PROJ_FOLD = True
MFMA_CONV_OUT = True
SHORTCUT_FOLD = os.environ.get("MSD_SHORTCUT_FOLD", "1") != "0"
SHORTCUT_FOLD_MAX_PIXELS = int(os.environ.get("MSD_SHORTCUT_FOLD_MAX_PIXELS", str(1 << 30)))
SHARE_CFG_PREFIX = os.environ.get("MSD_SHARE_CFG_PREFIX", "1") != "0"
W_CHUNK_MAJOR = os.environ.get("MSD_W_CHUNK_MAJOR", "1") != "0"
MFMA_TEMB_PROJ = os.environ.get("MSD_MFMA_TEMB_PROJ", "1") != "0"
XATTN_FUSED = os.environ.get("MSD_XATTN_FUSED", "1") != "0"
XATTN_FUSED_D160 = os.environ.get("MSD_XATTN_FUSED_D160", "0") != "0"


class Emitter:

    def __init__(self, plan: Plan, W: Dict[str, torch.Tensor], step_ptr=None):
        self.p, self.W, self.step_ptr = plan, W, step_ptr
        plan.keep.append(W)

    def w_layout(self, key: str) -> int:
        lay = getattr(self.W, "layout", None)
        return lay(key) if lay is not None else (1 if W_CHUNK_MAJOR else 0)

    def conv(self, x, name, N, ksize=1, stride=1, upsample=False, act=ops.ACT_NONE, residual: Optional[Act] = None,
             rowvec=None, out_dtype=ops.OUT_BF16, bias=True, wkey=None, split=None, out: Optional[Act] = None,
             asym_pad: bool = False, ln_out: bool = False, ln_in: Optional[tuple] = None, extra=None) -> Act:
        p = self.p
        x0, x1 = (x if isinstance(x, tuple) else (x, None))
        cin = x0.C + (x1.C if x1 is not None else 0)
        hl, wl = (2 * x0.H, 2 * x0.W) if upsample else (x0.H, x0.W)
        pad = 1 if ksize == 3 else 0
        pad_lead, pad_end = ((0, 1) if asym_pad else (pad, pad))
        ho, wo = (hl + pad_lead + pad_end - ksize) // stride + 1, (wl + pad_lead + pad_end - ksize) // stride + 1
        n_out = N // 2 if act == ops.ACT_GEGLU else N
        M = x0.B * ho * wo
        nk = ksize * ksize * (cin // 64)
        can_split = not (split is not None or act == ops.ACT_GEGLU)
        e0, e1 = (extra if isinstance(extra, tuple) else (extra, None))
        cx = 0 if e0 is None else e0.C + (e1.C if e1 is not None else 0)
        nk += cx // 64
        tile_m, tile_n, sk, stages = tuning.lookup(x0.B, x0.H, x0.W, cin, N, ksize, stride, upsample, M, nk, can_split, cx)
        if ln_out or ln_in is not None:
            sk = 1
        if sk > 1:
            p.ws_floats = max(p.ws_floats, sk * M * N)
        if out is None and split is None:
            esz = 4 if out_dtype == ops.OUT_F32 else 2
            out = Act(p.alloc(M * n_out * esz), x0.B, ho, wo, n_out)
        kw = dict(a0=x0.buf, a1=None if x1 is None else x1.buf, c1=0 if x1 is None else x1.C,
                  w=self.W[(wkey or name) + ".w"], out=out.buf if out is not None else None, batch=x0.B, h_in=x0.H,
                  w_in=x0.W, c0=x0.C, N=N, ksize=ksize, stride=stride, upsample=upsample,
                  bias=self.W[(wkey or name) + ".b"] if bias else None, act=act, out_dtype=out_dtype,
                  residual=None if residual is None else residual.buf, res_ld=None if residual is None else residual.C,
                  workspace=p.ws if sk > 1 else None, workspace_floats=sk * M * N if sk > 1 else 0, splitk=sk,
                  tile_m=tile_m, tile_n=tile_n, stages=stages, pad=pad_lead, pad_end=pad_end,
                  step_ptr=self.step_ptr if rowvec is not None else None, w_layout=self.w_layout((wkey or name) + ".w"), name=name)
        if e0 is not None:
            kw.update(a2=e0.buf, c2=e0.C, a3=None if e1 is None else e1.buf, c3=0 if e1 is None else e1.C)
        if ln_in is not None:
            wn = wkey or name
            kw.update(w=self.W[wn + ".lnw"], bias=self.W[wn + ".lnb"], ln_in=ln_in[0], ln_in_slots=ln_in[1],
                      ln_colsum=self.W[wn + ".lncs"], ln_eps=EPS, w_layout=self.w_layout(wn + ".lnw"))
        if tuning.form_of(tile_m, tile_n, stages).family == "wreg":
            wk = (wkey or name) + (".lnw" if ln_in is not None else ".w")
            frag = getattr(self.W, "fragment_major", None)
            if frag is not None:
                kw.update(w=frag(wk), w_layout=2)
            elif self.W[wk] is None:
                kw.update(w=None, w_layout=2)
            else:
                from . import packing
                src = self.W[wk]
                if self.w_layout(wk) == 1:
                    raise ValueError(f"{wk}: the wreg form needs packing.PackedWeights (a chunk-major tensor in a plain mapping cannot be re-laid)")
                kw.update(w=packing.fragment_major(src), w_layout=2)
        if ln_out:
            slots = ops.conv_gemm_ln_slots(N=N, tile_n=tile_n, tile_m=tile_m, ksize=ksize, act=act)
            out.ln = (p.alloc(M * slots * 8), slots)
            kw.update(ln_out=out.ln[0], ln_out_slots=slots)
        if rowvec is not None:
            kw.update(rowvec=rowvec[0], rv_step_stride=rowvec[1], rv_batch_stride=rowvec[2])
        if split is not None:
            ns0, ns1, out0, out1, out2, out2_ld = split
            kw.update(out=out0, out_ld=max(ns0, 4), split=(ns0, ns1, out1, ns1, out2, out2_ld))
        p.rec(ops.conv_gemm, **kw)
        return out

    def widen(self, x: Act, copies: int, name: str) -> Act:
        if copies == 1:
            return x
        nbytes = x.B * x.H * x.W * x.C * 2
        assert x.buf.nbytes >= copies * nbytes
        self.p.rec(ops.replicate, src=x.buf, dst=x.buf, nbytes=nbytes, copies=copies, name=name + ".replicate")
        return Act(x.buf, x.B * copies, x.H, x.W, x.C)

    def group_norm(self, x, name, silu: bool) -> Act:
        p = self.p
        x0, x1 = (x if isinstance(x, tuple) else (x, None))
        C = x0.C + (x1.C if x1 is not None else 0)
        out = p.act(x0.B, x0.H, x0.W, C)
        p.rec(ops.group_norm, x0=x0.buf, x1=None if x1 is None else x1.buf, c1=0 if x1 is None else x1.C,
              gamma=self.W[name + ".g"], beta=self.W[name + ".b"], stats=p.gn_stats_slot(x0.B), partials=p.gn_partials, out=out.buf, batch=x0.B,
              hw=x0.H * x0.W, c0=x0.C, silu=silu, eps=EPS, sync=p.gn_sync, name=name)
        return out

    def layer_norm(self, x: Act, name) -> Act:
        out = self.p.act(x.B, x.H, x.W, x.C)
        self.p.rec(ops.layer_norm, x=x.buf, gamma=self.W[name + ".g"], beta=self.W[name + ".b"], out=out.buf, rows=x.M,
                   c=x.C, eps=EPS, name=name)
        return out

    def res_block(self, x, name, cout, temb=None, free_input=False, out_copies: int = 1) -> Act:
        p = self.p
        x0 = x[0] if isinstance(x, tuple) else x
        cin = sum(a.C for a in x) if isinstance(x, tuple) else x.C
        g1 = self.group_norm(x, name + ".norm1", silu=True)
        h = self.conv(g1, name + ".conv1", cout, ksize=3, rowvec=temb)
        p.free(g1)
        g2 = self.group_norm(h, name + ".norm2", silu=True)
        p.free(h)
        fold = SHORTCUT_FOLD and (temb is None or x0.H * x0.W < SHORTCUT_FOLD_MAX_PIXELS)
        head = None
        if out_copies > 1:
            wide = p.act(x0.B * out_copies, x0.H, x0.W, cout)
            head = Act(wide.buf, x0.B, x0.H, x0.W, cout)
        if cin != cout and fold and (name + ".conv2sc.w") in self.W:
            out = self.conv(g2, name + ".conv2sc", cout, ksize=3, extra=x, out=head)
            p.free(g2)
        else:
            if cin != cout:
                res = self.conv(x, name + ".conv_shortcut", cout, ksize=1)
            else:
                assert not isinstance(x, tuple)
                res = x0
            out = self.conv(g2, name + ".conv2", cout, ksize=3, residual=res, out=head)
            p.free(g2)
            if res is not x0:
                p.free(res)
        if out_copies > 1:
            out = self.widen(out, out_copies, name)
        if free_input:
            for a in (x if isinstance(x, tuple) else (x,)):
                p.free(a)
        return out

    def attentions(self, x: Act, name, ctx_kv, ctx_len, heads=8, free_input=False, shared: int = 1, perturbed: int = 0) -> Act:
        p = self.p
        x_all = x
        if not 0 <= perturbed <= x.B or (perturbed and shared > 1):
            raise ValueError(f"{name}: {perturbed} perturbed rows of {x.B} (shared = {shared})")
        if shared > 1:
            assert x.B % shared == 0
            x = Act(x.buf, x.B // shared, x.H, x.W, x.C)
        B, H, Wd, C = x.B, x.H, x.W, x.C
        S = H * Wd
        d = C // heads
        tb = name + ".transformer_blocks.0"
        fold = LN_FOLD and (tb + ".attn1.qkv.lnw") in self.W
        g = self.group_norm(x, name + ".norm", silu=False)
        t0 = self.conv(g, name + ".proj_in", C, ln_out=fold)
        p.free(g)
        q, k = p.act(B, H, Wd, C), p.act(B, H, Wd, C)
        sp = (S + 7) // 8 * 8
        vt = p.alloc(B * C * sp * 2)
        if fold:
            self.conv(t0, tb + ".attn1.qkv", 3 * C, bias=False, split=(C, C, q.buf, k.buf, vt, sp), ln_in=t0.ln)
            p.free(t0.ln[0])
        else:
            n1 = self.layer_norm(t0, tb + ".norm1")
            self.conv(n1, tb + ".attn1.qkv", 3 * C, bias=False, split=(C, C, q.buf, k.buf, vt, sp))
            p.free(n1)
        a1 = p.act(B, H, Wd, C)
        if perturbed < B:
            p.rec(ops.attention, q=q.buf, k=k.buf, vt=vt, out=a1.buf, batch=B - perturbed, heads=heads, head_dim=d, s=S, t=S, q_ld=C,
                  k_ld=C, vt_ld=sp, o_ld=C, scale=d ** -0.5, q_prescaled=True, name=tb + ".attn1")
        if perturbed:
            p.rec(ops.attention_identity, vt=vt.at((B - perturbed) * C * sp * 2), out=a1.buf.at((B - perturbed) * S * C * 2),
                  batch=perturbed, channels=C, s=S, vt_ld=sp, o_ld=C, name=tb + ".attn1.identity")
        p.free(q, k, vt)
        if shared > 1:
            t1_wide = p.act(B * shared, H, Wd, C)
            t1 = self.conv(a1, tb + ".attn1.to_out.0", C, residual=t0, ln_out=fold, out=Act(t1_wide.buf, B, H, Wd, C))
            p.free(a1, t0)
            ln = t1.ln
            t1 = self.widen(t1, shared, tb + ".attn1.to_out.0")
            if ln is not None:
                nb_ln = B * H * Wd * ln[1] * 8
                ln_wide = p.alloc(shared * nb_ln)
                p.rec(ops.replicate, src=ln[0], dst=ln_wide, nbytes=nb_ln, copies=shared, name=tb + ".attn1.to_out.0.ln.replicate")
                p.free(ln[0])
                t1.ln = (ln_wide, ln[1])
            x, B = x_all, B * shared
        else:
            t1 = self.conv(a1, tb + ".attn1.to_out.0", C, residual=t0, ln_out=fold)
            p.free(a1, t0)
        kc, vtc, tp = ctx_kv[tb + ".attn2"]
        a2 = p.act(B, H, Wd, C)
        if fold and XATTN_FUSED and heads == 8 and (d in (40, 80) or (d == 160 and XATTN_FUSED_D160)) and ctx_len <= 96:
            wn = tb + ".attn2.to_q"
            p.rec(ops.cross_attention_q, x=t1.buf, ln_in=t1.ln[0], ln_in_slots=t1.ln[1], wq=self.W[wn + ".lnw"],
                  ln_colsum=self.W[wn + ".lncs"], bias=self.W[wn + ".lnb"], k=kc, vt=vtc, out=a2.buf, batch=B, heads=heads,
                  head_dim=d, s=S, t=ctx_len, k_ld=C, vt_ld=tp, o_ld=C, ln_eps=EPS, w_layout=self.w_layout(wn + ".lnw"),
                  name=tb + ".attn2")
            p.free(t1.ln[0])
        else:
            if fold:
                q2 = self.conv(t1, tb + ".attn2.to_q", C, bias=False, ln_in=t1.ln)
                p.free(t1.ln[0])
            else:
                n2 = self.layer_norm(t1, tb + ".norm2")
                q2 = self.conv(n2, tb + ".attn2.to_q", C, bias=False)
# ... 349 lines not shown
```

### minsdtf_amd/layout.py

```python
from __future__ import annotations

from dataclasses import dataclass, field, replace
from typing import List, NamedTuple, Optional, Tuple

import numpy as np

from .weights import UNET_HEADS

KERAS, ROWS, VEC = "keras", "rows", "vec"


class Flags(NamedTuple):
    chunk_major: bool = True
    mfma_temb_proj: bool = True


DIRECT = {
    "conv_in", "conv_out", "time_embedding.linear_1", "time_embedding.linear_2",
    "post_quant_conv", "decoder.conv_in", "decoder.conv_out", "encoder.conv_in", "quant_conv",
} | {f"input_hint_block.{i}" for i in range(7)}

STACKS = {
    ".attn1.to_q": (("to_q", "to_k", "to_v"), "qkv"),
    ".attn2.to_k": (("to_k", "to_v"), "kv"),
    ".query": (("query", "key", "value"), "qkv"),
    ".self_attn.q_proj": (("q_proj", "k_proj", "v_proj"), "qkv"),
}
_STACKED = tuple(first[: first.rindex(".") + 1] + m for first, (members, _) in STACKS.items() for m in members)

LATENT_SCALE = 0.18215


def q_prescale(c_out: int) -> np.float32:
    return np.float32((c_out // UNET_HEADS) ** -0.5 * 1.4426950408889634)


@dataclass
class Part:
    layer: str
    row_off: int = 0
    col_off: int = 0
    qscale: Optional[float] = None
    colscale: Optional[str] = None
    rowmap: bool = False
    ffproj_top: bool = False
    rows: Optional[int] = None


@dataclass
class Packed:
    key: str
    store: str
    shape: Tuple[int, ...]
    parts: List[Part] = field(default_factory=list)
    how: str = "w"
    chunk_major: bool = False
    norm: Optional[str] = None
    colsum: Optional[str] = None
    lnb: Optional[Tuple[str, str]] = None

    @property
    def dtype(self) -> str:
        return "bfloat16" if self.store == ROWS else "float32"

    @property
    def stored_shape(self) -> Tuple[int, ...]:
        return (self.shape[1] // 64, self.shape[0], 64) if self.chunk_major else self.shape

    @property
    def sources(self) -> set:
        return {p.layer for p in self.parts}


def layout(specs, flags: Flags = Flags()) -> List[Packed]:
    shape = {(s.name, s.kind): tuple(s.shape) for s in specs}
    out: List[Packed] = []

    def nk(n):
        s = shape.get((n, "conv_w"))
        return (s[3], s[0] * s[1] * s[2]) if s else shape[(n, "dense_w")][::-1]

    def rows(key, parts, **kw) -> Packed:
        n = max(p.row_off + nk(p.layer)[0] for p in parts)
        k = max(p.col_off + nk(p.layer)[1] for p in parts)
        out.append(Packed(key, ROWS, (n, k), parts, chunk_major=flags.chunk_major and k % 64 == 0, **kw))
        return out[-1]

    def keras(key, parts):
        conv = shape.get((parts[0].layer, "conv_w"))
        kh, kw, cin = conv[:3] if conv else (1, 1, shape[(parts[0].layer, "dense_w")][0])
        n = max(p.row_off + (p.rows or nk(p.layer)[0]) for p in parts)
        out.append(Packed(key, KERAS, (kh, kw, cin, n), parts))

    def vec(key, how, parts):
        kind = how if how in ("gamma", "beta") else "bias"
        n = sum(p.rows or shape[(p.layer, kind)][0] for p in (parts[:1] if how in ("bias_sum", "ffproj_b") else parts))
        out.append(Packed(key, VEC, (n,), parts, how=how))

    def fold(w_key, parts, norm, bias=()):
        if (norm, "gamma") not in shape:
            return
        base = w_key[: -len(".w")]
        e = rows(base + ".lnw", [replace(p, colscale=norm + ".g") for p in parts], norm=norm, colsum=base + ".lncs",
                 lnb=(base + ".lnb", norm + ".b"))
        out.append(Packed(base + ".lncs", VEC, e.shape[:1], how="lncs"))
        out.append(Packed(base + ".lnb", VEC, e.shape[:1], list(bias), how="lnb"))

    tproj = [s.name for s in specs if s.kind == "dense_w" and s.name.endswith(".time_emb_proj")]
    for n in dict.fromkeys(s.name for s in specs):
        has = lambda kind, n=n: (n, kind) in shape
        if has("embedding"):
            out.append(Packed(n, VEC, shape[(n, "embedding")], [Part(n)], how="embedding"))
        elif has("gamma"):
            vec(n + ".g", "gamma", [Part(n)])
            vec(n + ".b", "beta", [Part(n)])
        elif n.endswith(".time_emb_proj"):
            if n == tproj[0]:
                parts, off = [], 0
                for m in tproj:
                    parts.append(Part(m, row_off=off))
                    off += nk(m)[0]
                (rows if flags.mfma_temb_proj else keras)("time_emb_proj_cat.w", parts)
                vec("time_emb_proj_cat.b", "bias", [Part(m) for m in tproj])
        elif n in DIRECT:
            keras(n + ".w", [Part(n)])
            vec(n + ".b", "bias", [Part(n)])
            if n == "conv_out" and has("conv_w") and shape[(n, "conv_w")][2] % 64 == 0:
                rows(n + ".m.w", [Part(n)])
                vec(n + ".m.b", "bias", [Part(n)])
            if n == "quant_conv":
                keras(n + ".mean.w", [Part(n, rows=4, qscale=np.float32(LATENT_SCALE))])
                vec(n + ".mean.b", "bias", [Part(n, rows=4, qscale=np.float32(LATENT_SCALE))])
        elif n.endswith(".ff.net.0.proj"):
            parts = [Part(n, rowmap=True)]
            rows(n + ".w", parts)
            vec(n + ".b", "bias", parts)
            fold(n + ".w", parts, n[: -len(".ff.net.0.proj")] + ".norm3", bias=parts)
        elif n.endswith(".attn2.to_q"):
            parts = [Part(n, qscale=q_prescale(nk(n)[0]))]
            rows(n + ".w", parts)
            fold(n + ".w", parts, n[: -len(".attn2.to_q")] + ".norm2")
        elif n.endswith(tuple(STACKS)):
            first = next(f for f in STACKS if n.endswith(f))
            members, stacked = STACKS[first]
            base = n[: n.rindex(".") + 1]
            members = [base + m for m in members]
            unet = first == ".attn1.to_q"
            parts = [Part(m, row_off=i * nk(m)[0], qscale=q_prescale(nk(m)[0]) if unet and i == 0 else None)
                     for i, m in enumerate(members)]
            rows(base + stacked + ".w", parts)
            if (members[0], "bias") in shape:
                vec(base + stacked + ".b", "bias", [Part(m) for m in members])
            if unet:
                fold(base + stacked + ".w", parts, n[: -len(first)] + ".norm1")
        elif n.endswith(_STACKED):
            pass
        else:
            rows(n + ".w", [Part(n)])
            if has("bias"):
                vec(n + ".b", "bias", [Part(n)])
            if n.endswith(".transformer_blocks.0.ff.net.2"):
                att = n[: -len(".transformer_blocks.0.ff.net.2")]
                if (att + ".proj_out", "conv_w") in shape:
                    rows(att + ".ffproj.w", [Part(n, ffproj_top=True), Part(att + ".proj_out", col_off=nk(n)[1])])
                    vec(att + ".ffproj.b", "ffproj_b", [Part(n), Part(att + ".proj_out")])
            elif n.endswith(".conv2"):
                rb = n[: -len(".conv2")]
                sc = rb + ".conv_shortcut"
                w2, ws = shape.get((n, "conv_w")), shape.get((sc, "conv_w"))
                if w2 and ws and w2[0] == 3 and ws[0] == 1 and ws[2] % 64 == 0:
                    rows(rb + ".conv2sc.w", [Part(n), Part(sc, col_off=nk(n)[1])])
                    vec(rb + ".conv2sc.b", "bias_sum", [Part(n), Part(sc)])
    return out
```

### minsdtf_amd/ops.py

```python
from __future__ import annotations

import ctypes as C
from typing import Optional

from . import _lib
from ._lib import ACT_GEGLU, ACT_NONE, ACT_QUICK_GELU, ACT_SILU, OUT_BF16, OUT_F32, OUT_U8


class Call:

    __slots__ = ("fn", "args", "name", "keep")

    def __init__(self, fn, args, name, keep=None):
        self.fn, self.args, self.name, self.keep = fn, args, name, keep

    def __call__(self, stream: int) -> None:
        rc = self.fn(*self.args, stream)
        if rc != 0:
            _lib.check(rc, self.name)


def _p(x) -> Optional[int]:
    if x is None:
        return None
    if isinstance(x, int):
        return x
    if hasattr(x, "ptr"):
        return x.ptr
    return x.data_ptr()


def conv_gemm(*, a0, w, out, batch, h_in, w_in, c0, N, a1=None, c1=0, ksize=1, stride=1, upsample=False, bias=None,
              rowvec=None, rv_step_stride=0, rv_batch_stride=0, step_ptr=None, residual=None, res_ld=None, act=ACT_NONE,
              out_dtype=OUT_BF16, out_ld=None, split=None, workspace=None, workspace_floats=0, splitk=1, tile_n=0,
              tile_m=0, stages=0, pad=None, pad_end=None, ln_in=None, ln_in_slots=0, ln_colsum=None, ln_out=None,
              ln_out_slots=0, ln_eps=1e-5, a2=None, c2=0, a3=None, c3=0, w_layout=0, name="conv_gemm") -> Call:
    lib = _lib.load()
    if pad is None:
        pad = 1 if ksize == 3 else 0
    if pad_end is None:
        pad_end = pad
    hl, wl = (2 * h_in, 2 * w_in) if upsample else (h_in, w_in)
    h_out = (hl + pad + pad_end - ksize) // stride + 1
    w_out = (wl + pad + pad_end - ksize) // stride + 1
    n_out = N // 2 if act == ACT_GEGLU else N
    s = _lib.MsdConvGemm()
    s.a0, s.a1, s.w = _p(a0), _p(a1), _p(w)
    s.bias, s.rowvec, s.step_ptr, s.residual = _p(bias), _p(rowvec), _p(step_ptr), _p(residual)
    s.out = _p(out)
    s.workspace, s.workspace_floats = _p(workspace), int(workspace_floats)
    s.batch, s.h_in, s.w_in, s.c0, s.c1 = batch, h_in, w_in, c0, c1
    s.h_out, s.w_out, s.ksize, s.stride, s.pad, s.upsample = h_out, w_out, ksize, stride, pad, int(bool(upsample))
    s.N, s.act, s.out_dtype = N, act, out_dtype
    s.out_ld = n_out if out_ld is None else out_ld
    s.res_ld = (n_out if res_ld is None else res_ld) if residual is not None else 0
    s.rv_step_stride, s.rv_batch_stride = rv_step_stride, rv_batch_stride
    if split is not None:
        ns0, ns1, out1, out1_ld, out2, out2_ld = split
        s.split_mode, s.ns0, s.ns1 = 1, ns0, ns1
        s.out1, s.out1_ld, s.out2, s.out2_ld = _p(out1), out1_ld, _p(out2), out2_ld
        if out_ld is None:
            s.out_ld = max(ns0, 4)
    s.splitk, s.tile_n, s.tile_m, s.stages = splitk, tile_n, tile_m, stages
    s.ln_in, s.ln_colsum, s.ln_out = _p(ln_in), _p(ln_colsum), _p(ln_out)
    s.ln_in_slots, s.ln_out_slots, s.ln_eps = ln_in_slots, ln_out_slots, float(ln_eps)
    s.a2, s.a3, s.c2, s.c3 = _p(a2), _p(a3), c2, c3
    s.w_layout = int(w_layout)
    return Call(lib.msd_conv_gemm, (C.byref(s),), name, keep=s)


def conv_gemm_ln_slots(*, N, tile_n, tile_m=0, ksize=1, act=ACT_NONE) -> int:
    lib = _lib.load()
    s = _lib.MsdConvGemm()
    s.N, s.tile_n, s.tile_m, s.ksize, s.act = N, tile_n, tile_m, ksize, act
    n = lib.msd_conv_gemm_ln_slots(C.byref(s))
    if n <= 0:
        _lib.check(n, "conv_gemm_ln_slots")
    return n


def conv_direct(*, x, w, out, batch, h_in, w_in, c_in, c_out, ksize=3, stride=1, bias=None, residual=None,
                in_batch_mod=None, in_dtype=OUT_BF16, out_dtype=OUT_BF16, act=ACT_NONE, act_in=False, in_scale=1.0,
                name="conv_direct") -> Call:
    lib = _lib.load()
    pad = 1 if ksize == 3 else 0
    s = _lib.MsdConvDirect()
    s.in_, s.w, s.bias, s.residual, s.out = _p(x), _p(w), _p(bias), _p(residual), _p(out)
    s.batch, s.in_batch_mod = batch, (batch if in_batch_mod is None else in_batch_mod)
    s.h_in, s.w_in, s.c_in = h_in, w_in, c_in
    s.h_out = (h_in + 2 * pad - ksize) // stride + 1
    s.w_out = (w_in + 2 * pad - ksize) // stride + 1
    s.c_out, s.ksize, s.stride, s.pad = c_out, ksize, stride, pad
    s.in_dtype, s.out_dtype, s.act, s.act_in, s.in_scale = in_dtype, out_dtype, act, int(bool(act_in)), float(in_scale)
    return Call(lib.msd_conv_direct, (C.byref(s),), name, keep=s)


GN_MAX_CHUNKS = 1024


GN_SYNC_WORDS_PER_SAMPLE = 16384


def group_norm(*, x0, gamma, beta, stats, partials, out, batch, hw, c0, x1=None, c1=0, silu=False, eps=1e-5,
               partials_floats=None, sync=None, sync_words=None, name="group_norm") -> Call:
    lib = _lib.load()
    s = _lib.MsdGroupNorm()
    s.x0, s.x1, s.gamma, s.beta, s.stats, s.out = _p(x0), _p(x1), _p(gamma), _p(beta), _p(stats), _p(out)
    s.partials = _p(partials)
    s.partials_floats = batch * GN_MAX_CHUNKS * 64 if partials_floats is None else partials_floats
    s.batch, s.hw, s.c0, s.c1, s.silu, s.eps = batch, hw, c0, c1, int(bool(silu)), float(eps)
    s.sync = _p(sync)
    s.sync_words = 0 if sync is None else (batch * GN_SYNC_WORDS_PER_SAMPLE if sync_words is None else sync_words)
    return Call(lib.msd_group_norm, (C.byref(s),), name, keep=s)


def layer_norm(*, x, gamma, beta, out, rows, c, eps=1e-5, name="layer_norm") -> Call:
    lib = _lib.load()
    return Call(lib.msd_layer_norm, (_p(x), _p(gamma), _p(beta), _p(out), rows, c, C.c_float(eps)), name)


def attention(*, q, k, vt, out, batch, heads, head_dim, s, t, q_ld, k_ld, vt_ld, o_ld, scale, causal=False,
              q_prescaled=False, workspace=None, workspace_floats=0, name="attention") -> Call:
    lib = _lib.load()
    a = _lib.MsdAttention()
    a.q, a.k, a.vt, a.out = _p(q), _p(k), _p(vt), _p(out)
    a.batch, a.heads, a.head_dim, a.s, a.t = batch, heads, head_dim, s, t
    a.q_ld, a.k_ld, a.vt_ld, a.o_ld, a.scale = q_ld, k_ld, vt_ld, o_ld, float(scale)
    a.causal = int(bool(causal))
    a.q_prescaled = int(bool(q_prescaled))
    a.workspace, a.workspace_floats = _p(workspace), int(workspace_floats)
    return Call(lib.msd_attention, (C.byref(a),), name, keep=a)


def cross_attention_q(*, x, ln_in, ln_in_slots, wq, ln_colsum, bias, k, vt, out, batch, heads, head_dim, s, t, k_ld, vt_ld, o_ld,
                      ln_eps=1e-5, w_layout=0, name="cross_attention_q") -> Call:
    lib = _lib.load()
    a = _lib.MsdCrossAttnQ()
    a.x, a.ln_in, a.wq, a.ln_colsum, a.bias, a.k, a.vt, a.out = _p(x), _p(ln_in), _p(wq), _p(ln_colsum), _p(bias), _p(k), _p(vt), _p(out)
    a.batch, a.heads, a.head_dim, a.s, a.t = batch, heads, head_dim, s, t
    a.k_ld, a.vt_ld, a.o_ld, a.ln_in_slots, a.ln_eps, a.w_layout = k_ld, vt_ld, o_ld, ln_in_slots, float(ln_eps), int(w_layout)
    return Call(lib.msd_cross_attention_q, (C.byref(a),), name, keep=a)


def softmax_rows(*, x, out, rows, cols, ld_in, ld_out, scale, name="softmax_rows") -> Call:
    lib = _lib.load()
    return Call(lib.msd_softmax_rows, (_p(x), _p(out), rows, cols, ld_in, ld_out, C.c_float(scale)), name)


def cfg_step(*, eps, latent, coef, step_ptr, batch, n, num_steps, guidance, guidance_rescale, advance=True,
             inpaint_init=None, inpaint_noise=None, inpaint_mask=None, step_noise=None, noise_coef=None,
             name="cfg_step") -> Call:
    lib = _lib.load()
    s = _lib.MsdCfgStep()
    s.eps, s.latent, s.coef, s.step_ptr = _p(eps), _p(latent), _p(coef), _p(step_ptr)
    s.inpaint_init, s.inpaint_noise, s.inpaint_mask = _p(inpaint_init), _p(inpaint_noise), _p(inpaint_mask)
    s.step_noise, s.noise_coef = _p(step_noise), _p(noise_coef)
    s.batch, s.n, s.num_steps = batch, n, num_steps
    s.guidance, s.guidance_rescale, s.advance = float(guidance), float(guidance_rescale), int(advance)
    return Call(lib.msd_cfg_step, (C.byref(s),), name, keep=s)


def sampler_step(*, eps, latent, coef, step_ptr, denoised_prev, batch, n, num_steps, guidance, guidance_rescale, advance=True,
                 inpaint_init=None, inpaint_noise=None, inpaint_mask=None, step_noise=None, name="sampler_step") -> Call:
    lib = _lib.load()
    s = _lib.MsdSamplerStep()
    s.eps, s.latent, s.coef, s.step_ptr = _p(eps), _p(latent), _p(coef), _p(step_ptr)
    s.inpaint_init, s.inpaint_noise, s.inpaint_mask = _p(inpaint_init), _p(inpaint_noise), _p(inpaint_mask)
    s.step_noise, s.denoised_prev = _p(step_noise), _p(denoised_prev)
    s.batch, s.n, s.num_steps = batch, n, num_steps
    s.guidance, s.guidance_rescale, s.advance = float(guidance), float(guidance_rescale), int(advance)
    return Call(lib.msd_sampler_step, (C.byref(s),), name, keep=s)


def latent_resample(*, x, out, wx, wy, batch, h_in, w_in, h_out, w_out, a=1.0, s=0.0, noise=None, name="latent_resample") -> Call:
    lib = _lib.load()
    r = _lib.MsdLatentResample()
    r.in_, r.out, r.noise, r.wx, r.wy = _p(x), _p(out), _p(noise), _p(wx), _p(wy)
    r.batch, r.h_in, r.w_in, r.h_out, r.w_out = int(batch), int(h_in), int(w_in), int(h_out), int(w_out)
    r.a, r.s = float(a), float(s)
    return Call(lib.msd_latent_resample, (C.byref(r),), name, keep=r)


def tile_consensus(*, tiles, canvas, wy, wx, ys, xs, th, tw, H, W, batch, mode=0, name="tile_consensus") -> Call:
    lib = _lib.load()
    ys, xs = [int(v) for v in ys], [int(v) for v in xs]
    if not 1 <= len(ys) <= _lib.TILE_MAX_VIEWS or not 1 <= len(xs) <= _lib.TILE_MAX_VIEWS:
        raise ValueError(f"tile_consensus: {len(ys)} x {len(xs)} views (1 .. {_lib.TILE_MAX_VIEWS} per axis)")
    t = _lib.MsdTileConsensus()
    t.tiles, t.canvas, t.wy, t.wx = _p(tiles), _p(canvas), _p(wy), _p(wx)
    t.ys[:len(ys)], t.xs[:len(xs)] = ys, xs
    t.rows, t.cols, t.th, t.tw, t.H, t.W, t.batch, t.mode = len(ys), len(xs), int(th), int(tw), int(H), int(W), int(batch), int(mode)
    return Call(lib.msd_tile_consensus, (C.byref(t),), name, keep=t)


def region_combine(*, eps, w, out, regions, batch, n, name="region_combine") -> Call:
    lib = _lib.load()
    s = _lib.MsdRegionCombine()
    s.eps, s.w, s.out = _p(eps), _p(w), _p(out)
    s.regions, s.batch, s.n = int(regions), int(batch), int(n)
    return Call(lib.msd_region_combine, (C.byref(s),), name, keep=s)


def attention_identity(*, vt, out, batch, channels, s, vt_ld, o_ld, name="attention_identity") -> Call:
    lib = _lib.load()
    a = _lib.MsdAttentionIdentity()
    a.vt, a.out = _p(vt), _p(out)
    a.batch, a.channels, a.s, a.vt_ld, a.o_ld = int(batch), int(channels), int(s), int(vt_ld), int(o_ld)
    return Call(lib.msd_attention_identity, (C.byref(a),), name, keep=a)


def add_bf16(*, a, b, out, n, name="add_bf16") -> Call:
    lib = _lib.load()
    return Call(lib.msd_add_bf16, (_p(a), _p(b), _p(out), n), name)


def add_f32_bf16(*, a, b, out, n, name="add_f32_bf16") -> Call:
    lib = _lib.load()
    return Call(lib.msd_add_f32_bf16, (_p(a), _p(b), _p(out), n), name)


def cast_f32_to_bf16(*, x, out, n, name="cast_f2b") -> Call:
# ... 60 lines not shown
```

### minsdtf_amd/packing.py

```python
from __future__ import annotations

from typing import Dict, List, NamedTuple, Optional, Tuple

import numpy as np
import torch

from .layout import KERAS, VEC, Packed


def _dev_bf16(t: torch.Tensor, device) -> torch.Tensor:
    return t.to(torch.bfloat16).contiguous().to(device)


class PackedWeights(dict):

    def __init__(self, *a, **kw):
        super().__init__(*a, **kw)
        self.chunk_major_keys = set()
        self._fragment = {}

    def layout(self, key: str) -> int:
        return 1 if key in self.chunk_major_keys else 0

    def to_chunk_major(self, key: str) -> None:
        t = self[key]
        if key in self.chunk_major_keys or t.dim() != 2 or t.shape[1] % 64:
            return
        self[key] = chunk_major(t)
        self.chunk_major_keys.add(key)


    def fragment_major(self, key: str) -> torch.Tensor:
        t = self._fragment.get(key)
        if t is None:
            w = self[key]
            if key in self.chunk_major_keys:
                w = w.permute(1, 0, 2).reshape(w.shape[1], -1)
            t = self._fragment[key] = fragment_major(w)
        return t


FRAGMENT_ROW_ORDER = (0, 1, 2, 3, 8, 9, 10, 11, 4, 5, 6, 7, 12, 13, 14, 15)


def fragment_major(w_nk: torch.Tensor) -> torch.Tensor:
    n, k = w_nk.shape
    assert n % 16 == 0 and k % 64 == 0, (n, k)
    order = torch.tensor(FRAGMENT_ROW_ORDER, device=w_nk.device)
    w = w_nk.reshape(n // 16, 16, k)[:, order, :]
    w = w.reshape(n // 16, 16, k // 64, 2, 4, 8)
    return w.permute(2, 0, 3, 4, 1, 5).contiguous()


def chunk_major(w_nk: torch.Tensor) -> torch.Tensor:
    n, k = w_nk.shape
    assert k % 64 == 0, (n, k)
    return w_nk.view(n, k // 64, 64).permute(1, 0, 2).contiguous()


def logical(w: np.ndarray) -> torch.Tensor:
    t = torch.from_numpy(np.ascontiguousarray(w, dtype=np.float32))
    return t.permute(3, 0, 1, 2).reshape(t.shape[3], -1) if t.dim() == 4 else t.t()


def pack_matrix(w: np.ndarray, device) -> torch.Tensor:
    return _dev_bf16(logical(w), device)


pack_conv = pack_dense = pack_matrix


def pack_dense_stack(ws, device) -> torch.Tensor:
    return _dev_bf16(torch.cat([logical(w) for w in ws], dim=0), device)


def geglu_row_order(n_half: int) -> np.ndarray:
    assert n_half % 16 == 0
    p = np.arange(2 * n_half)
    grp, within = p // 32, p % 32
    return np.where(within < 16, grp * 16 + within, n_half + grp * 16 + (within - 16))


def pack_geglu(w_io: np.ndarray, b: np.ndarray, device):
    n_half = w_io.shape[1] // 2
    order = geglu_row_order(n_half)
    return _dev_bf16(logical(w_io)[torch.from_numpy(order)], device), dev_f32(np.asarray(b)[order], device)


def fold_layer_norm(w_oi: torch.Tensor, bias, gamma: np.ndarray, beta: np.ndarray, device):
    g = torch.from_numpy(np.ascontiguousarray(gamma, dtype=np.float32))
    bt = torch.from_numpy(np.ascontiguousarray(beta, dtype=np.float32))
    wf = (w_oi * g[None, :]).to(torch.bfloat16)
    colsum = wf.to(torch.float64).sum(dim=1).to(torch.float32)
    c = (w_oi.to(torch.float64) @ bt.to(torch.float64)).to(torch.float32)
    if bias is not None:
        c = c + torch.from_numpy(np.ascontiguousarray(bias, dtype=np.float32))
    return wf.contiguous().to(device), colsum.contiguous().to(device), c.contiguous().to(device)


def dev_f32(a: np.ndarray, device) -> torch.Tensor:
    return torch.from_numpy(np.ascontiguousarray(a, dtype=np.float32)).to(device)


class Masters(NamedTuple):
    layer: Dict[str, torch.Tensor]
    top: Dict[str, torch.Tensor]
    vec: Dict[str, torch.Tensor]


def _weight(named, layer) -> np.ndarray:
    w = named.get((layer, "conv_w"))
    return w if w is not None else named[(layer, "dense_w")]


def _as_1x1(w: np.ndarray) -> np.ndarray:
    return np.asarray(w, np.float64).reshape(w.shape[-2], w.shape[-1])


def _matrix(e: Packed, named) -> torch.Tensor:
    blocks = []
    for i, p in enumerate(e.parts):
        if p.ffproj_top:
            m = logical((np.asarray(_weight(named, p.layer), np.float64) @ _as_1x1(_weight(named, e.parts[i + 1].layer)))
                        .astype(np.float32))
        else:
            m = logical(_weight(named, p.layer))
        if p.qscale is not None:
            m = m * float(p.qscale)
        if p.rowmap:
            m = m[torch.from_numpy(geglu_row_order(m.shape[0] // 2))]
        blocks.append(m)
    return blocks[0] if len(blocks) == 1 else torch.cat(blocks, dim=1 if e.parts[1].col_off else 0)


def _keras(e: Packed, named) -> np.ndarray:
    blocks = []
    for p in e.parts:
        w = _weight(named, p.layer)
        w = w.reshape(1, 1, *w.shape) if w.ndim == 2 else w
        if p.rows:
            w = np.asarray(w, dtype=np.float32)[..., :p.rows]
        blocks.append(w if p.qscale is None else w * p.qscale)
    return blocks[0] if len(blocks) == 1 else np.concatenate(blocks, axis=-1)


def _vector(e: Packed, named) -> Optional[np.ndarray]:
    kind = e.how if e.how in ("gamma", "beta", "embedding") else "bias"
    blocks = []
    for p in e.parts:
        v = np.asarray(named[(p.layer, kind)])
        if p.rowmap:
            v = v[geglu_row_order(len(v) // 2)]
        if p.rows:
            v = np.asarray(v, dtype=np.float32)[:p.rows]
        blocks.append(v if p.qscale is None else v * p.qscale)
    if e.how == "bias_sum":
        return np.asarray(blocks[0], np.float32) + np.asarray(blocks[1], np.float32)
    if e.how == "ffproj_b":
        wp = _as_1x1(_weight(named, e.parts[1].layer))
        return (np.asarray(blocks[0], np.float64) @ wp + np.asarray(blocks[1], np.float64)).astype(np.float32)
    return None if not blocks else blocks[0] if len(blocks) == 1 else np.concatenate(blocks)


def pack(layout: List[Packed], named, device, keep=None) -> Tuple[PackedWeights, Optional[Masters]]:
    W = PackedWeights()
    by_key = {e.key: e for e in layout}
    masters = None if keep is None else Masters({}, {}, {})
    kept = lambda e: masters is not None and not e.sources.isdisjoint(keep)
    for e in layout:
        if e.how in ("lncs", "lnb"):
            continue
        if e.store == VEC:
            W[e.key] = dev_f32(_vector(e, named), device)
            if e.how == "ffproj_b" and kept(e):
                masters.vec[e.key] = W[e.key].clone()
            continue
        if e.store == KERAS:
            W[e.key] = dev_f32(_keras(e, named), device)
            continue
        m = _matrix(e, named)
        if e.parts[0].ffproj_top and kept(e):
            masters.top[e.parts[0].layer] = m[:, : e.parts[1].col_off].contiguous().to(device)
        if e.norm is None:
            W[e.key] = _dev_bf16(m, device)
        else:
            lncs, lnb = e.colsum, e.lnb[0]
            W[e.key], W[lncs], W[lnb] = fold_layer_norm(m.contiguous(), _vector(by_key[lnb], named), named[(e.norm, "gamma")],
                                                        named[(e.norm, "beta")], device)
            if kept(e):
                masters.vec[lncs], masters.vec[lnb] = W[lncs].clone(), W[lnb].clone()
        if e.chunk_major:
            W.to_chunk_major(e.key)
    for n in keep or ():
        masters.layer[n] = logical(_weight(named, n)).contiguous().to(device)
    return W, masters


def save_packed(W: PackedWeights, path: str, meta: dict = None) -> None:
    import os

    blob = {"meta": dict(meta or {}), "chunk_major": sorted(W.chunk_major_keys),
            "tensors": {k: (t.detach().cpu() if isinstance(t, torch.Tensor) else t) for k, t in W.items()}}
    tmp = f"{path}.tmp.{os.getpid()}"
    torch.save(blob, tmp)
    os.replace(tmp, path)


def load_packed(path: str, device, meta: dict = None) -> PackedWeights:
    blob = torch.load(path, map_location="cpu", mmap=True, weights_only=True)
    if meta is not None and blob["meta"] != dict(meta):
        raise ValueError(f"{path}: packed for {blob['meta']}, wanted {dict(meta)}")
    W = PackedWeights({k: (t.to(device) if isinstance(t, torch.Tensor) else t) for k, t in blob["tensors"].items()})
    W.chunk_major_keys = set(blob["chunk_major"])
    return W
```

### minsdtf_amd/tuning.py

```python
from __future__ import annotations

import json
import os
import re
from typing import Dict, NamedTuple, Optional, Tuple

_PATH = os.path.join(os.path.dirname(os.path.abspath(__file__)), "conv_tuning.json")
_table: Optional[Dict[str, list]] = None
_families: Optional[Dict[str, Dict[int, list]]] = None

TILES = ((128, 128, 0), (128, 64, 0), (64, 64, 0), (64, 128, 0), (256, 128, 0),
         (128, 128, 4), (64, 64, 8), (64, 128, 5), (128, 64, 5), (128, 80, 0), (128, 80, 4),
         (64, 64, 14), (128, 64, 13), (64, 128, 13),
         (128, 128, 23), (128, 128, 24), (128, 64, 24), (64, 128, 24),
         (128, 160, 0))
HALO_TILES = ((1128, 64, 0), (1128, 128, 0), (1256, 128, 0), (1128, 80, 0), (1256, 80, 0),
              (1128, 64, 8), (1128, 128, 6), (1128, 80, 8), (1256, 80, 5), (2128, 64, 0), (2128, 80, 0),
              (1128, 64, 33), (1128, 64, 34), (1128, 80, 33), (2128, 64, 33),
              (1128, 64, 63), (1128, 80, 63),
              (1128, 64, 93), (1128, 80, 93),
              (1128, 64, 153), (1128, 64, 158), (1128, 128, 153), (1128, 128, 156), (1256, 128, 153), (1128, 80, 158),
              (1256, 80, 153), (1256, 80, 155))


WREG_TILES = ((4128, 128, 3), (4128, 128, 4), (4128, 64, 3), (4128, 64, 4), (4064, 128, 3), (4064, 128, 4), (4064, 256, 3), (4064, 256, 4),
              (4064, 64, 4), (4256, 64, 3), (4128, 128, 13),
              (4064, 64, 23), (4064, 64, 24), (4064, 128, 23), (4064, 128, 24), (4064, 256, 23), (4128, 64, 23), (4128, 128, 23),
              (4256, 128, 13), (4256, 128, 14))


BIG_TILES = ((5256, 256, 0), (5256, 160, 0), (5256, 160, 1), (5256, 160, 2), (5256, 128, 0), (5256, 128, 1), (5128, 256, 0), (5128, 256, 1))
BIG_TILES_CHUNK_MAJOR = ((5256, 256, 10), (5256, 160, 10), (5256, 160, 11), (5256, 128, 10), (5128, 256, 10))
BIG_TILES_HALO_IMAGE = ((5256, 160, 20), (5256, 128, 20), (5256, 128, 21))
BIG_MIN_ROWS = 4096
HALO_IMAGE_MIN_ROWS = 256


Form = NamedTuple("Form", [("family", str), ("rows", int), ("cols", int), ("code", int), ("chunk_major", bool), ("variant", int), ("th", int), ("name", str)])


def _family(tile_m: int) -> Optional[str]:
    return next(fam for base, fam in ((6000, None), (5000, "big"), (4000, "wreg"), (3000, "rowpanel"), (1000, "halo"), (tile_m, "tile")) if tile_m >= base)


def form_of(tile_m: int, tile_n: int, stages: int = 0) -> Form:
    fam, rows, walk = _family(tile_m), tile_m % 1000, 2 if stages >= 20 else 1 if stages >= 10 else 0
    if fam is None:
        raise ValueError(f"tile_m {tile_m} names no kernel form")
    if fam == "big":
        name = f"staged halo 16x16 x{tile_n}" if walk == 2 else f"big {rows}x{tile_n}" + (" chunk-major" if walk else "")
        return Form("bighalo" if walk == 2 else fam, rows, tile_n, stages - 10 * walk, walk > 0, 0, 0, name)
    if fam == "wreg":
        return Form(fam, rows, tile_n, stages, False, (1 if stages % 20 >= 10 else 0) + (2 if walk == 2 else 0), 0, f"wreg {rows}x{tile_n}" + (" 2K/stage" if walk == 2 else ""))
    if fam == "rowpanel":
        return Form(fam, rows, tile_n, stages, False, 0, 0, f"row panel x{tile_n}")
    if fam == "halo":
        step = " rotated 1 tap" if stages >= 150 else " rotated 3 taps" if stages >= 90 else " 3 taps + loaders" if stages >= 60 else " 3 taps/step" if stages >= 30 else ""
        return Form(fam, rows, tile_n, stages, True, tile_m // 2000, rows // 16, f"halo {rows // 16}x16" + (" (8 waves)" if tile_m >= 2000 else "") + f" x{tile_n}{step}")
    return Form(fam, tile_m, tile_n, stages, False, walk, 0, f"tile {tile_m}x{tile_n}" + ("", " (8 waves)", " (64x64/wave)")[walk])


is_halo, is_rowpanel, is_wreg, is_big = (lambda tile_m, _fam=fam: _family(tile_m) == _fam for fam in ("halo", "rowpanel", "wreg", "big"))


def wreg_nj(tile_m: int, tile_n: int, stages: int) -> int:
    f = form_of(tile_m, tile_n, stages)
    return tile_n // 16 // (8 if (f.variant & 1 and f.rows != 256) else 4)


ROWPANEL_ROWS = {320: (3128,), 640: (3128,)}
ROWPANEL_COLS = (64, 96, 128, 160, 192, 320, 480, 640, 960)


def shape_key(batch, h_in, w_in, cin, N, ksize, stride, upsample, allow_split=True, cx=0) -> str:
    return (f"{batch}x{h_in}x{w_in}x{cin}->{N}k{ksize}s{stride}u{int(bool(upsample))}{'' if allow_split else 'n'}"
            f"{'+x' + str(cx) if cx else ''}")


def _load() -> Dict[str, list]:
    global _table, _families
    if _table is None:
        try:
            with open(_PATH) as f:
                _table = json.load(f)
        except (OSError, ValueError):
            _table = {}
        ov = os.environ.get("MSD_TUNE_OVERRIDE")
        if ov:
            if ov.startswith("@"):
                with open(ov[1:]) as f:
                    ov = f.read()
            _table.update({k: list(v) + [0.0] for k, v in json.loads(ov).items()})
        _families = {}
        for key, ent in _table.items():
            b, rest = key.split("x", 1)
            _families.setdefault(rest, {})[int(b)] = ent
    return _table


def heuristic(M: int, N: int, nk: int, allow_split: bool) -> Tuple[int, int, int, int]:
    bn = 128 if (N % 128 == 0 or N > 1024) else 64
    bm = 128
    if M <= 64:
        bm = 64
    tiles = ((M + bm - 1) // bm) * ((N + bn - 1) // bn)
    sk = 1
    if allow_split and tiles < 160 and nk >= 32:
        sk = max(1, min((256 + tiles - 1) // tiles, nk // 8, 16))
    return bm, bn, sk, 0


def _ceil_div(a: int, b: int) -> int:
    return -(-a // b)


def shape_class(h_in, w_in, cin, N, ksize, stride, upsample, allow_split, cx=0) -> Tuple[str, int, int]:
    hl, wl = (2 * h_in, 2 * w_in) if upsample else (h_in, w_in)
    pad = 1 if ksize == 3 else 0
    ho, wo = (hl + 2 * pad - ksize) // stride + 1, (wl + 2 * pad - ksize) // stride + 1
    hw_out = ho * wo
    nkc = cin // 64
    nk = ksize * ksize * nkc + cx // 64
    tile16 = stride == 1 and hl % 16 == 0 and wl % 16 == 0
    walk = "tap"
    if ksize == 3 and stride == 1:
        if cx == 0 and not upsample and w_in % 16 == 0 and h_in % 8 == 0 and hw_out >= 256:
            walk = "chunk"
        elif cx == 0 and upsample and tile16 and h_in * w_in >= 256:
            walk = "chunk"
        elif cx and w_in % 16 == 0 and h_in % 8 == 0 and hw_out >= 256:
            walk = "chunk_sc"
    sk = 1
    if allow_split:
        if walk != "tap":
            wgs = _ceil_div(hw_out, 128) * _ceil_div(N, 64)
            if wgs < 256 and hw_out < 4096:
                sk = max(1, min(_ceil_div(512, 2 * wgs), nkc // (2 if N < 64 else 6)))
        elif ksize == 3 or nk >= 32:
            if ksize == 3 and hw_out < 4096:
                sk = max(1, min(_ceil_div(96, max(1, int(hw_out ** 0.5))), nk // 8, 16))
            elif ksize == 1 and hw_out < 1024:
                sk = max(1, min(_ceil_div(48, max(1, int(hw_out ** 0.5))), nk // 8, 16))
        elif nk >= 16 and N <= 2048:
            sk = 4 if hw_out <= 64 else 2 if hw_out <= 144 else 1
    ln_tile = 64 if (ksize == 1 and allow_split and cx == 0 and cin == N) else 0
    return walk, sk, ln_tile


def shape_config(batch, h_in, w_in, cin, N, ksize, stride, upsample, M, nk, allow_split, cx=0) -> Tuple[int, int, int, int]:
    walk, sk, ln_tile = shape_class(h_in, w_in, cin, N, ksize, stride, upsample, allow_split, cx)
    hl, wl = (2 * h_in, 2 * w_in) if upsample else (h_in, w_in)
    tile16 = stride == 1 and hl % 16 == 0 and wl % 16 == 0
    wide = 128 if (N % 128 == 0 or N > 1024) else 64
    if walk == "chunk_sc":
        wgs16 = batch * (hl // 16) * (wl // 16) * _ceil_div(N, 128) * sk if tile16 else 0
        if N >= 128 and wgs16 >= 128:
            return 5256, (160 if (N % 160 == 0 and M >= 32768 and allow_split) else 128), sk, 20
        if M <= 4096 or N < 80:
            return 1128, 64, sk, 0
        return 1128, (80 if (N % 80 == 0 and allow_split) else 64), sk, 93
    if walk == "chunk":
        wgs16 = batch * (hl // 16) * (wl // 16) * _ceil_div(N, 128) * sk if tile16 else 0
        if upsample:
            if tile16:
                return 5256, (160 if (N % 160 == 0 and M >= 32768) else 128), sk, 20
            return 5256, 128, sk, 10
        if N >= 128 and wgs16 >= 128:
            return 5256, (160 if (N % 160 == 0 and M >= 32768 and allow_split) else 128), sk, 20
        if M <= 4096 or N < 80:
            return 2128, 64, sk, (33 if M <= 16384 else 0)
        return 1128, (80 if (N % 80 == 0 and allow_split) else 64), sk, 93
    if ln_tile:
        return (64, 64, sk, 0) if M <= 2048 else (128, 64, sk, 13)
    if ksize == 1 and not allow_split:
        if cin in ROWPANEL_ROWS and N % 32 == 0 and M >= 4096 and stride == 1 and not upsample and not cx:
            panels = _ceil_div(M, 128)
            cols = [c for c in ROWPANEL_COLS if N % c == 0]
            fit = [c for c in cols if panels * (N // c) >= 512]
            if cols:
                return ROWPANEL_ROWS[cin][0], (max(fit) if fit else min(cols)), 1, 0
        if M <= 512:
            return 64, 64, 1, 14
        if M <= 4096 or N <= 64:
            return 128, wide, 1, 0
        return 256, 128, 1, 0
    if ksize == 1 and nk < 32:
        if N > 4096:
            return (64, 128, sk, 0) if M <= 2048 else (128, 128, sk, 0)
        if M <= 2048:
            return 64, 64, sk, 0
        if M < 16384 or N < 128:
            return 128, 64, sk, 13
        return 5256, (160 if N % 160 == 0 else 128), sk, (1 if N % 160 == 0 else 0)
    if M <= 256:
        return 64, 64, sk, 14
    if M <= 1024:
        return (4064, 128, sk, 23) if N % 128 == 0 else (128, 64, sk, 0)
    if M <= 4096 or N < 128:
        return (128, 128, sk, 4) if wide == 128 else (128, 64, sk, 0)
    if M < 8192:
        return 256, 128, sk, 0
    return 5256, (160 if N % 160 == 0 else 128), sk, (1 if N % 160 == 0 else 0)


def lookup(batch, h_in, w_in, cin, N, ksize, stride, upsample, M, nk, allow_split, cx=0) -> Tuple[int, int, int, int]:
    key = shape_key(batch, h_in, w_in, cin, N, ksize, stride, upsample, allow_split, cx)
    ent = _load().get(key)
    if ent is None:
        fam = _families.get(key.split("x", 1)[1])
        if fam:
            ent = fam[min(fam, key=lambda b: (abs(b - batch) / (b + batch), b))]
            if int(ent[0]) == 256 and M < 1024:
                ent = [128] + list(ent[1:])
            if is_big(int(ent[0])) and M < BIG_MIN_ROWS:
                big = form_of(int(ent[0]), int(ent[1]), int(ent[3]) if len(ent) > 4 else 0)
                if big.family == "bighalo" and cx:
                    if w_in % 16 == 0 and h_in % 8 == 0:
                        ent = [1128, 80 if (N % 80 == 0 and M > 4096) else 64, int(ent[2]), 93 if M > 4096 else 0, 0.0]
                elif big.chunk_major and not upsample and stride == 1 and w_in % 16 == 0 and h_in % 8 == 0:
                    ent = [1128, 80 if N % 80 == 0 else 64, int(ent[2]), 0, 0.0]
                elif big.chunk_major:
                    ent = [5256, 128, int(ent[2]), 10, 0.0]
                else:
                    ent = [128, 128 if N % 128 == 0 else 64, int(ent[2]), 0, 0.0]
    if ent is not None:
        bm, bn, sk = int(ent[0]), int(ent[1]), int(ent[2])
        stages = int(ent[3]) if len(ent) > 4 else 0
        if not allow_split:
            sk = 1
        return bm, bn, sk, stages
    if os.environ.get("MSD_SHAPE_CONFIG", "1") == "0":
        return heuristic(M // max(1, batch), N, nk, allow_split)
    return shape_config(batch, h_in, w_in, cin, N, ksize, stride, upsample, M, nk, allow_split, cx)


def numerics_class(ksize: int, tile_m: int, tile_n: int, splitk: int, ln_producer: bool = True, stages: int = 0) -> Tuple[bool, int, int]:
    f = form_of(tile_m, tile_n, stages)
    cols = 64 if f.family == "rowpanel" else 0 if f.family in ("big", "bighalo") and f.chunk_major else tile_n
    return (f.chunk_major, splitk, cols if (ksize == 1 and ln_producer) else 0)


def key_is_ln_producer(key: str) -> bool:
    m = re.match(r"\d+x\d+x\d+x(\d+)->(\d+)k(\d)s\du[01](n?)(\+x\d+)?$", key)
    if m is None:
        return True
    cin, n, ks, nos, cx = m.groups()
    return ks == "1" and nos != "n" and cx is None and cin == n
```

Before: 10.27 images/s.

## Add phase-decomposed 2x upsample conv path with folded 2x2 weights

```diff
diff --git a/include/minsdtf_hip.h b/include/minsdtf_hip.h
--- a/include/minsdtf_hip.h
+++ b/include/minsdtf_hip.h
@@ -76,6 +76,7 @@
     const void* a3;
     int32_t c2, c3;
     int32_t w_layout;
+    const void* w_phase;
 } MsdConvGemm;
 
 MSD_API int msd_conv_gemm_ln_slots(const MsdConvGemm* p);
diff --git a/minsdtf_amd/_lib.py b/minsdtf_amd/_lib.py
--- a/minsdtf_amd/_lib.py
+++ b/minsdtf_amd/_lib.py
@@ -32,6 +32,7 @@
         ("ln_in", C.c_void_p), ("ln_colsum", C.c_void_p), ("ln_out", C.c_void_p),
         ("ln_in_slots", C.c_int32), ("ln_out_slots", C.c_int32), ("ln_eps", C.c_float),
         ("a2", C.c_void_p), ("a3", C.c_void_p), ("c2", C.c_int32), ("c3", C.c_int32), ("w_layout", C.c_int32),
+        ("w_phase", C.c_void_p),
     ]
 
 
diff --git a/minsdtf_amd/csrc/conv_big.hip b/minsdtf_amd/csrc/conv_big.hip
--- a/minsdtf_amd/csrc/conv_big.hip
+++ b/minsdtf_amd/csrc/conv_big.hip
@@ -442,9 +442,10 @@
 #endif
 }
 
-template <int BN, int WGM, int WGN, int NBW>
+template <int BN, int WGM, int WGN, int NBW, bool PHS = false>
 __global__ __launch_bounds__(512) void conv_bighalo_kernel(CG_HOT_PARAMS, const CGArgs p) {
     CG_HOT_UNPACK;
+    constexpr int NT = PHS ? 4 : 9;
     constexpr int BM = 256, HW_ = 18, HROWS = 18 * 18, HPAD = 336;
     static_assert(WGM * WGN == 8 && BN % 32 == 0 && BN % (WGN * 16) == 0, "tile");
     constexpr int WMT = BM / WGM, WNT = BN / WGN, MI = WMT / 16, NJ = WNT / 16, IHS = MI / 2;
@@ -454,7 +455,9 @@
     constexpr int LEAD = NBW - 1;
     static_assert(LEAD >= 1 && LEAD <= 3, "weight steps in flight (the halo RAW rule needs <= 3)");
     static_assert(2 * H_BYTES + NBW * W_BYTES <= 160 * 1024, "LDS");
-    constexpr int NWAIT = LEAD + WR * (LEAD - 1);
+    constexpr int HS = PHS ? (LEAD == 3 ? 3 : 2) : 1;
+    static_assert(!PHS || (6 / HS - 1 <= 4 - LEAD && WR - W0 >= 1), "phase form: the next chunk's halo is older than its first step's weights");
+    constexpr int NWAIT = PHS ? (LEAD - 1) * (WR + HS) : LEAD + WR * (LEAD - 1);
     extern __shared__ __attribute__((aligned(16))) char smem[];
     const uint32_t lds0 = (uint32_t)(size_t)(__attribute__((address_space(3))) char*)smem;
 
@@ -464,14 +467,16 @@
     const int grp = wave >> 2;
     const int r = lane & 15, g = lane >> 4;
     MSD_STAMP(0);
-    const int ups = p.upsample ? 1 : 0;
+    const int ups = (!PHS && p.upsample) ? 1 : 0;
     const int Hl = p.h_in << ups, Wl = p.w_in << ups;
     const int tiles_x = Wl >> 4, tps = tiles_x * (Hl >> 4);
     const int tile = xcd_remap(blockIdx.x, hot_tiles_m * hot_tiles_n);
     const int tdiv = hot_m_fast ? hot_tiles_m : hot_tiles_n;
     const int tq = udiv_magic(tile, tdiv, hot_mg_tdiv), tr = tile - tq * tdiv;
     const int tile_n = hot_m_fast ? tq : tr;
-    const int tmi = hot_m_fast ? tr : tq;
+    const int tmi_ = hot_m_fast ? tr : tq;
+    const int py = PHS ? ((tmi_ >> 1) & 1) : 0, px = PHS ? (tmi_ & 1) : 0;
+    const int tmi = PHS ? (tmi_ >> 2) : tmi_;
     const int b = udiv_magic(tmi, tps, p.mg_tps);
     const int trem = tmi - b * tps;
     const int tyi = udiv_magic(trem, tiles_x, p.mg_tx);
@@ -479,7 +484,7 @@
     const int n0 = tile_n * BN;
     const int c_begin = blockIdx.y * hot_nk_per;
     const int nch = min(p.nkc, c_begin + hot_nk_per) - c_begin;
-    const int nkt = nch * 9;
+    const int nkt = nch * NT;
 
     const int cpos = lane & 7, lr8 = lane >> 3;
     const char* zero = reinterpret_cast<const char*>(g_zero_page) + cpos * 16;
@@ -488,7 +493,7 @@
     for (int k = 0; k < 6; ++k) {
         const int hrow = k < 5 ? 64 * k + 8 * wave + lr8 : 320 + 2 * wave + (lr8 & 1);
         const int hy = (hrow * 3641) >> 16, hx = hrow - hy * HW_;
-        const int iy = ty0 + hy - 1, ix = tx0 + hx - 1;
+        const int iy = ty0 + hy - 1 + py, ix = tx0 + hx - 1 + px;
         const bool ok = hrow < HROWS && (unsigned)iy < (unsigned)Hl && (unsigned)ix < (unsigned)Wl;
         const int pix = (b * p.h_in + (min(max(iy, 0), Hl - 1) >> ups)) * p.w_in + (min(max(ix, 0), Wl - 1) >> ups);
         hpix[k] = ok ? pix : -1;
@@ -529,12 +534,13 @@
         else if constexpr (k == 5) dma16m(reinterpret_cast<const void*>(a), ldsH5_wave + boff, 0xFFFFull);
         else dma16(zero, lds0 + boff + 328u * 128u);
     };
+    const char* wbase = PHS ? reinterpret_cast<const char*>(p.wph) + (size_t)(2 * py + px) * (size_t)(4 * p.nkc) * hot_w_ks : reinterpret_cast<const char*>(hot_w);
     auto issue_w = [&](auto LO_, auto HI_, uint32_t koff, int ib) {
         constexpr int LO = decltype(LO_)::value, HI = decltype(HI_)::value;
         const uint32_t boff = (uint32_t)ib * (uint32_t)W_BYTES;
 #pragma unroll
         for (int k = LO; k < HI; ++k) {
-            const char* wb = reinterpret_cast<const char*>(hot_w) + koff;
+            const char* wb = wbase + koff;
             if (k < WRF) dma16s(wb, woff[k], ldsW_wave + boff + (uint32_t)k * 8192u);
             else dma16sm(wb, woff[k], ldsWh_wave + boff + (uint32_t)k * 8192u, 0xFFFFFFFFull);
         }
@@ -560,12 +566,19 @@
         fire_halo(std::integral_constant<int, 5>{}, halo_addr(std::integral_constant<int, 5>{}, t, true), 0);
 #pragma unroll
         for (int tt = 0; tt < LEAD; ++tt) {
-            issue_w(std::integral_constant<int, 0>{}, std::integral_constant<int, WR>{}, w_koff(c_begin, tt), tt);
-            fire_halo(std::integral_constant<int, 6>{}, 0, 1);
+            if constexpr (PHS) {
+                issue_w(std::integral_constant<int, 0>{}, std::integral_constant<int, W0>{}, w_koff(c_begin, tt), tt);
+#pragma unroll
+                for (int q = 0; q < HS; ++q) fire_halo(std::integral_constant<int, 6>{}, 0, 1);
+                issue_w(std::integral_constant<int, W0>{}, std::integral_constant<int, WR>{}, w_koff(c_begin, tt), tt);
+            } else {
+                issue_w(std::integral_constant<int, 0>{}, std::integral_constant<int, WR>{}, w_koff(c_begin, tt), tt);
+                fire_halo(std::integral_constant<int, 6>{}, 0, 1);
+            }
         }
     }
     MSD_STAMP(1);
-    wait_vmcnt<1 + (LEAD - 1) * (WR + 1)>();
+    wait_vmcnt<PHS ? (LEAD - 1) * (WR + HS) : 1 + (LEAD - 1) * (WR + 1)>();
     __builtin_amdgcn_s_barrier();
     if (grp == 1) __builtin_amdgcn_s_barrier();
 
@@ -629,6 +642,7 @@
     int rb = 0, ib = LEAD % NBW;
     prep_frag(0, 0, 0, 0);
     uint64_t ph = 0;
+    uint64_t php[PHS ? HS : 1] = {};
     ChunkA nx = chunk_a(c_begin);
     for (int c = 0; c < nch; ++c) {
         const int hb = c & 1;
@@ -640,10 +654,10 @@
 #endif
         auto step = [&](auto TAP_) {
             constexpr int TAP = decltype(TAP_)::value;
-            constexpr int ky = TAP / 3, kx = TAP - ky * 3;
-            constexpr int TAPW = (TAP + LEAD) % 9, CW = (TAP + LEAD) / 9;
-            constexpr int TAPN = (TAP + 1) % 9;
-            const int rem = nkt - 1 - (c * 9 + TAP);
+            constexpr int ky = PHS ? TAP / 2 : TAP / 3, kx = PHS ? TAP % 2 : TAP - ky * 3;
+            constexpr int TAPW = (TAP + LEAD) % NT, CW = (TAP + LEAD) / NT;
+            constexpr int TAPN = (TAP + 1) % NT;
+            const int rem = nkt - 1 - (c * NT + TAP);
             const uint32_t koff = w_koff(c_begin + c + CW, TAPW);
             load_w(rb);
             load_a();
@@ -651,32 +665,60 @@
             if (rem >= LEAD) issue_w(std::integral_constant<int, 0>{}, std::integral_constant<int, W0>{}, koff, ib);
             mfma_slot_open();
             prep_frag(1, ky, kx, hb);
-            if constexpr (TAP < 6) ph = halo_addr(std::integral_constant<int, TAP>{}, nx, has_next);
+            if constexpr (PHS) {
+                if constexpr (TAP * HS < 6) php[0] = halo_addr(std::integral_constant<int, (TAP * HS < 6 ? TAP * HS : 0)>{}, nx, has_next);
+                if constexpr (TAP * HS + 1 < 6) php[1] = halo_addr(std::integral_constant<int, (TAP * HS + 1 < 6 ? TAP * HS + 1 : 0)>{}, nx, has_next);
+                if constexpr (HS > 2 && TAP * HS + 2 < 6) php[HS - 1] = halo_addr(std::integral_constant<int, (TAP * HS + 2 < 6 ? TAP * HS + 2 : 0)>{}, nx, has_next);
+            } else {
+                if constexpr (TAP < 6) ph = halo_addr(std::integral_constant<int, (TAP < 6 ? TAP : 0)>{}, nx, has_next);
+            }
             mfma_part(std::integral_constant<int, 0>{});
-            if constexpr (TAP < 6) asm volatile("" : "+v"(ph));
+            if constexpr (PHS) {
+#pragma unroll
+                for (int q = 0; q < HS; ++q) asm volatile("" : "+v"(php[q]));
+            } else {
+                if constexpr (TAP < 6) asm volatile("" : "+v"(ph));
+            }
             mfma_slot_close();
             load_a();
             __builtin_amdgcn_sched_barrier(0);
-            if (rem >= LEAD) issue_w(std::integral_constant<int, W0>{}, std::integral_constant<int, WR>{}, koff, ib);
-            if constexpr (TAP < 6) fire_halo(std::integral_constant<int, TAP>{}, ph, hb ^ 1);
-            else fire_halo(std::integral_constant<int, 6>{}, 0, hb ^ 1);
-            if (rem >= LEAD) wait_vmcnt<NWAIT>();
-            else if (rem >= 1) big_wait(LEAD + WR * max(0, min(LEAD - 1, rem - 1)));
+            if constexpr (PHS) {
+                if constexpr (TAP * HS < 6) fire_halo(std::integral_constant<int, (TAP * HS < 6 ? TAP * HS : 6)>{}, php[0], hb ^ 1);
+                else fire_halo(std::integral_constant<int, 6>{}, 0, hb ^ 1);
+                if constexpr (TAP * HS + 1 < 6) fire_halo(std::integral_constant<int, (TAP * HS + 1 < 6 ? TAP * HS + 1 : 6)>{}, php[1], hb ^ 1);
+                else fire_halo(std::integral_constant<int, 6>{}, 0, hb ^ 1);
+                if constexpr (HS > 2) {
+                    if constexpr (TAP * HS + 2 < 6) fire_halo(std::integral_constant<int, (TAP * HS + 2 < 6 ? TAP * HS + 2 : 6)>{}, php[HS - 1], hb ^ 1);
+                    else fire_halo(std::integral_constant<int, 6>{}, 0, hb ^ 1);
+                }
+                if (rem >= LEAD) issue_w(std::integral_constant<int, W0>{}, std::integral_constant<int, WR>{}, koff, ib);
+                if (rem >= LEAD) wait_vmcnt<NWAIT>();
+                else if (rem >= 1) big_wait((LEAD - 1) * HS + WR * max(0, min(LEAD - 1, rem - 1)));
+            } else {
+                if (rem >= LEAD) issue_w(std::integral_constant<int, W0>{}, std::integral_constant<int, WR>{}, koff, ib);
+                if constexpr (TAP < 6) fire_halo(std::integral_constant<int, (TAP < 6 ? TAP : 6)>{}, ph, hb ^ 1);
+                else fire_halo(std::integral_constant<int, 6>{}, 0, hb ^ 1);
+                if (rem >= LEAD) wait_vmcnt<NWAIT>();
+                else if (rem >= 1) big_wait(LEAD + WR * max(0, min(LEAD - 1, rem - 1)));
+            }
             mfma_slot_open();
-            prep_frag(0, TAPN / 3, TAPN % 3, TAP == 8 ? hb ^ 1 : hb);
+            prep_frag(0, PHS ? TAPN / 2 : TAPN / 3, PHS ? TAPN % 2 : TAPN % 3, TAP == NT - 1 ? hb ^ 1 : hb);
             mfma_part(std::integral_constant<int, 1>{});
             mfma_slot_close();
             if (++rb == NBW) rb = 0;
             if (++ib == NBW) ib = 0;
         };
         step(std::integral_constant<int, 0>{}); step(std::integral_constant<int, 1>{}); step(std::integral_constant<int, 2>{});
-        step(std::integral_constant<int, 3>{}); step(std::integral_constant<int, 4>{}); step(std::integral_constant<int, 5>{});
-        step(std::integral_constant<int, 6>{}); step(std::integral_constant<int, 7>{}); step(std::integral_constant<int, 8>{});
+        step(std::integral_constant<int, 3>{});
+        if constexpr (!PHS) {
+            step(std::integral_constant<int, 4>{}); step(std::integral_constant<int, 5>{});
+            step(std::integral_constant<int, 6>{}); step(std::integral_constant<int, 7>{}); step(std::integral_constant<int, 8>{});
+        }
     }
     if (grp == 0) __builtin_amdgcn_s_barrier();
     wait_vmcnt<0>();
 
-    const int nxc = p.nk - p.nk_main;
+    const int nxc = PHS ? 0 : p.nk - p.nk_main;
     if (nxc > 0) {
         const int eps = (nxc + p.nslices - 1) / p.nslices;
         const int e0 = min(nxc, (int)blockIdx.y * eps), e1 = min(nxc, e0 + eps);
@@ -724,8 +766,9 @@
         constexpr int h = decltype(H_)::value;
         int mrow[EC];
 #pragma unroll
-        for (int i = 0; i < EC; ++i) mrow[i] = (b * Hl + ty0 + wm * MI + h * EC + i) * Wl + tx0;
-        cg_epilogue<EC, NJ, true, false>(p, acc[h], mrow, n0 + wn * WNT, r, g);
+        for (int i = 0; i < EC; ++i)
+            mrow[i] = PHS ? (b * 2 * Hl + 2 * (ty0 + wm * MI + h * EC + i) + py) * (2 * Wl) + 2 * tx0 + px : (b * Hl + ty0 + wm * MI + h * EC + i) * Wl + tx0;
+        cg_epilogue<EC, NJ, true, false>(p, acc[h], mrow, n0 + wn * WNT, PHS ? 2 * r : r, g);
     };
     epilogue_chunk(std::integral_constant<int, 0>{});
     if constexpr (EH > 1) epilogue_chunk(std::integral_constant<int, 1>{});
@@ -779,6 +822,9 @@
 #define X(bn, wgm, wgn, nbw, code)                                                                                            \
     if (e == hipSuccess)                                                                                                      \
         e = hipFuncSetAttribute(reinterpret_cast<const void*>(&conv_bighalo_kernel<bn, wgm, wgn, nbw>),                       \
+                                hipFuncAttributeMaxDynamicSharedMemorySize, bighalo_lds(bn, nbw));                            \
+    if (e == hipSuccess)                                                                                                      \
+        e = hipFuncSetAttribute(reinterpret_cast<const void*>(&conv_bighalo_kernel<bn, wgm, wgn, nbw, true>),                 \
                                 hipFuncAttributeMaxDynamicSharedMemorySize, bighalo_lds(bn, nbw));
     MSD_BIGHALO_CFGS(X)
 #undef X
@@ -829,8 +875,12 @@
     const dim3 grid(a.tiles_m * a.tiles_n, slices);
 #define X(bn_, wgm, wgn, nbw, code_)                                                                                          \
     if (f.cols == bn_ && f.code == code_) {                                                                                   \
-        hipLaunchKernelGGL((conv_bighalo_kernel<bn_, wgm, wgn, nbw>), grid, dim3(512), bighalo_lds(bn_, nbw), stream,         \
-                           CG_HOT_ARGS(a), a);                                                                                \
+        if (f.family == CG_BIGPHASE)                                                                                          \
+            hipLaunchKernelGGL((conv_bighalo_kernel<bn_, wgm, wgn, nbw, true>), grid, dim3(512), bighalo_lds(bn_, nbw),       \
+                               stream, CG_HOT_ARGS(a), a);                                                                    \
+        else                                                                                                                  \
+            hipLaunchKernelGGL((conv_bighalo_kernel<bn_, wgm, wgn, nbw>), grid, dim3(512), bighalo_lds(bn_, nbw), stream,     \
+                               CG_HOT_ARGS(a), a);                                                                            \
         return MSD_OK;                                                                                                        \
     }
     MSD_BIGHALO_CFGS(X)
diff --git a/minsdtf_amd/csrc/conv_common.h b/minsdtf_amd/csrc/conv_common.h
--- a/minsdtf_amd/csrc/conv_common.h
+++ b/minsdtf_amd/csrc/conv_common.h
@@ -19,6 +19,7 @@
     float ln_eps, ln_inv_k;
     int kmajor;
     uint32_t w_rs, w_ks;
+    const bf16_t* wph;
 };
 #include "conv_form.h"
 
diff --git a/minsdtf_amd/csrc/conv_form.h b/minsdtf_amd/csrc/conv_form.h
--- a/minsdtf_amd/csrc/conv_form.h
+++ b/minsdtf_amd/csrc/conv_form.h
@@ -7,6 +7,7 @@
     CG_WREG,
     CG_BIG,
     CG_BIGHALO,
+    CG_BIGPHASE,
     CG_NONE
 };
 struct CGForm {
@@ -19,13 +20,13 @@
     int variant;
     int th;
 };
-static inline CGForm cg_decode_form(int tile_m, int tile_n, int stages) {
+static inline CGForm cg_decode_form(int tile_m, int tile_n, int stages, bool phase = false) {
     const int walk = stages >= 20 ? 2 : stages >= 10 ? 1 : 0;
     CGForm f = {CG_TILE, tile_m >= 0 && tile_m < 6000, tile_m, tile_n, stages, false, 0, 0};
     if (tile_m >= 6000) f.family = CG_NONE;
     else if (tile_m < 1000) f.variant = walk;
     else if (tile_m >= 5000) {
-        f.family = walk == 2 ? CG_BIGHALO : CG_BIG;
+        f.family = walk == 2 ? (phase ? CG_BIGPHASE : CG_BIGHALO) : CG_BIG;
         f.rows = tile_m - 5000; f.code = stages - 10 * walk; f.chunk_major = walk > 0;
     } else if (tile_m >= 3000) {
         f.family = tile_m >= 4000 ? CG_WREG : CG_ROWPANEL;
@@ -36,7 +37,7 @@
     }
     return f;
 }
-static inline bool cg_is_big(const CGForm& f) { return f.family == CG_BIG || f.family == CG_BIGHALO; }
+static inline bool cg_is_big(const CGForm& f) { return f.family == CG_BIG || f.family == CG_BIGHALO || f.family == CG_BIGPHASE; }
 
 int msd_conv_halo_launch(const CGArgs& a, const CGForm& f, int slices, hipStream_t stream);
 bool msd_conv_rowpanel_eligible(const CGArgs& a, int rows, int wg_cols);
diff --git a/minsdtf_amd/csrc/conv_gemm.hip b/minsdtf_amd/csrc/conv_gemm.hip
--- a/minsdtf_amd/csrc/conv_gemm.hip
+++ b/minsdtf_amd/csrc/conv_gemm.hip
@@ -460,9 +460,12 @@
     }
     if ((long long)a.N * a.K * 2 >= (1ll << 32) - 4096) MSD_FAIL(MSD_E_UNSUPPORTED, "conv_gemm: an operand of 4 GB or more");
     if (q->w_layout < 0 || q->w_layout > 2) MSD_FAIL(MSD_E_ARG, "conv_gemm: w_layout %d", q->w_layout);
-    const CGForm f = cg_decode_form(q->tile_m, q->tile_n, q->stages);
+    const CGForm f = cg_decode_form(q->tile_m, q->tile_n, q->stages, q->w_phase != nullptr);
     if (!f.valid) MSD_FAIL(MSD_E_ARG, "conv_gemm: tile_m %d names no kernel form", q->tile_m);
-    const bool wreg = f.family == CG_WREG, big = cg_is_big(f), bighalo = f.family == CG_BIGHALO;
+    const bool wreg = f.family == CG_WREG, big = cg_is_big(f), phase = f.family == CG_BIGPHASE, bighalo = f.family == CG_BIGHALO || phase;
+    if (q->w_phase && !phase)
+        MSD_FAIL(MSD_E_ARG, "conv_gemm: a phase image (w_phase) is read by the staged-halo big form only (tile_m 5256, stages 20 + code), not tile_m %d stages %d", q->tile_m, q->stages);
+    a.wph = (const bf16_t*)q->w_phase;
     if (big) {
         if (f.chunk_major && (q->ksize != 3 || (q->a2 && !bighalo)))
             MSD_FAIL(MSD_E_UNSUPPORTED, "conv_gemm: the chunk-major walk of the big-tile form is for 3x3 convs (with a shortcut operand: on the staged-halo variant only)");
@@ -472,6 +475,8 @@
             const int up = q->upsample ? 2 : 1;
             if (q->stride != 1 || q->pad != 1 || q->h_out != up * q->h_in || q->w_out != up * q->w_in || (q->h_out % 16) || (q->w_out % 16))
                 MSD_FAIL(MSD_E_UNSUPPORTED, "conv_gemm: the halo-image big-tile form runs 3x3 / stride 1 / pad 1 convs on output images of whole 16 x 16-pixel tiles (%d x %d)", q->h_out, q->w_out);
+            if (phase && (!q->upsample || q->ksize != 3 || (q->h_in % 16) || (q->w_in % 16) || q->a2 || q->w_layout != 1 || q->split_mode || q->rowvec || !msd_aligned16(q->w_phase)))
+                MSD_FAIL(MSD_E_UNSUPPORTED, "conv_gemm: the phase form runs nearest x2 + 3x3 convs on input images of whole 16 x 16-pixel tiles (%d x %d), w_layout 1, no shortcut operand, no split epilogue, no rowvec", q->h_in, q->w_in);
         } else if (!msd_conv_big_nj(f))
             MSD_FAIL(MSD_E_UNSUPPORTED, "conv_gemm: no big-tile configuration %d x %d code %d", f.rows, f.cols, f.code);
         if (q->ln_out) MSD_FAIL(MSD_E_UNSUPPORTED, "conv_gemm: the big-tile form has no LayerNorm-producer epilogue (ln_out)");
@@ -536,9 +541,11 @@
         if ((rc = cg_dense_form(q, a, false, &dense)) || (rc = cg_hot_check(a))) return rc;
         rc = wreg ? msd_conv_wreg_launch(a, run, slices, dense, stream) : msd_conv_big_launch(a, run, slices, dense, stream);
         break;
+    case CG_BIGPHASE:
     case CG_BIGHALO: {
-        const int ty = a.h_out / 16, tx = a.w_out / 16;
-        cg_set_tiles(a, a.batch * ty * tx, run.cols, ty * tx, tx);
+        const bool ph = run.family == CG_BIGPHASE;
+        const int ty = (ph ? a.h_in : a.h_out) / 16, tx = (ph ? a.w_in : a.w_out) / 16;
+        cg_set_tiles(a, a.batch * ty * tx * (ph ? 4 : 1), run.cols, ty * tx, tx);
         if ((rc = cg_hot_check(a))) return rc;
         rc = msd_conv_bighalo_launch(a, run, slices, stream);
         break;
diff --git a/minsdtf_amd/engine.py b/minsdtf_amd/engine.py
--- a/minsdtf_amd/engine.py
+++ b/minsdtf_amd/engine.py
@@ -301,6 +301,7 @@
 MFMA_TEMB_PROJ = os.environ.get("MSD_MFMA_TEMB_PROJ", "1") != "0"
 XATTN_FUSED = os.environ.get("MSD_XATTN_FUSED", "1") != "0"
 XATTN_FUSED_D160 = os.environ.get("MSD_XATTN_FUSED_D160", "0") != "0"
+PHASE_CONV = os.environ.get("MSD_PHASE_CONV", "1") != "0"
 
 
 class Emitter:
@@ -348,6 +349,14 @@
                   step_ptr=self.step_ptr if rowvec is not None else None, w_layout=self.w_layout((wkey or name) + ".w"), name=name)
         if e0 is not None:
             kw.update(a2=e0.buf, c2=e0.C, a3=None if e1 is None else e1.buf, c3=0 if e1 is None else e1.C)
+        if upsample and tuning.form_of(tile_m, tile_n, stages).family == "bighalo" and \
+                tuning.phase_form(x0.H, x0.W, cin, N, ksize, stride, upsample, can_split, cx):
+            pm = getattr(self.W, "phase_major", None)
+            if not PHASE_CONV:
+                kw.update(w_phase=False)
+            elif pm is not None:
+                wph = pm((wkey or name) + ".w")
+                kw.update(w_phase=wph if wph is not None else False)
         if ln_in is not None:
             wn = wkey or name
             kw.update(w=self.W[wn + ".lnw"], bias=self.W[wn + ".lnb"], ln_in=ln_in[0], ln_in_slots=ln_in[1],
diff --git a/minsdtf_amd/layout.py b/minsdtf_amd/layout.py
--- a/minsdtf_amd/layout.py
+++ b/minsdtf_amd/layout.py
@@ -35,6 +35,15 @@
     return np.float32((c_out // UNET_HEADS) ** -0.5 * 1.4426950408889634)
 
 
+PHASE_TAPS = (((0,), (1, 2)), ((0, 1), (2,)))
+UPSAMPLER_CONV = ".upsamplers.0.conv"
+
+
+def phase_shape(n: int, k: int) -> Tuple[int, ...]:
+    cin = k // 9
+    return (4, 4 * cin // 64, n, 64)
+
+
 @dataclass
 class Part:
     layer: str
@@ -58,6 +67,7 @@
     norm: Optional[str] = None
     colsum: Optional[str] = None
     lnb: Optional[Tuple[str, str]] = None
+    phase: bool = False
 
     @property
     def dtype(self) -> str:
@@ -156,7 +166,9 @@
         elif n.endswith(_STACKED):
             pass
         else:
-            rows(n + ".w", [Part(n)])
+            e = rows(n + ".w", [Part(n)])
+            conv = shape.get((n, "conv_w"))
+            e.phase = bool(n.endswith(UPSAMPLER_CONV) and conv and conv[0] == 3 and conv[1] == 3 and conv[2] % 64 == 0 and e.chunk_major)
             if has("bias"):
                 vec(n + ".b", "bias", [Part(n)])
             if n.endswith(".transformer_blocks.0.ff.net.2"):
diff --git a/minsdtf_amd/ops.py b/minsdtf_amd/ops.py
--- a/minsdtf_amd/ops.py
+++ b/minsdtf_amd/ops.py
@@ -34,7 +34,7 @@
               rowvec=None, rv_step_stride=0, rv_batch_stride=0, step_ptr=None, residual=None, res_ld=None, act=ACT_NONE,
               out_dtype=OUT_BF16, out_ld=None, split=None, workspace=None, workspace_floats=0, splitk=1, tile_n=0,
               tile_m=0, stages=0, pad=None, pad_end=None, ln_in=None, ln_in_slots=0, ln_colsum=None, ln_out=None,
-              ln_out_slots=0, ln_eps=1e-5, a2=None, c2=0, a3=None, c3=0, w_layout=0, name="conv_gemm") -> Call:
+              ln_out_slots=0, ln_eps=1e-5, a2=None, c2=0, a3=None, c3=0, w_layout=0, w_phase=None, name="conv_gemm") -> Call:
     lib = _lib.load()
     if pad is None:
         pad = 1 if ksize == 3 else 0
@@ -66,7 +66,19 @@
     s.ln_in_slots, s.ln_out_slots, s.ln_eps = ln_in_slots, ln_out_slots, float(ln_eps)
     s.a2, s.a3, s.c2, s.c3 = _p(a2), _p(a3), c2, c3
     s.w_layout = int(w_layout)
-    return Call(lib.msd_conv_gemm, (C.byref(s),), name, keep=s)
+    if w_phase is None and upsample and ksize == 3 and stride == 1 and a2 is None and w_layout == 1 and split is None and rowvec is None:
+        from . import tuning
+        cin = c0 + c1
+        if tuning.form_of(tile_m, tile_n, stages).family == "bighalo" and tuning.phase_form(h_in, w_in, cin, N, ksize, stride, upsample, True, 0):
+            import torch
+            if isinstance(w, torch.Tensor):
+                from . import packing
+                w_phase = packing.phase_major_of_packed(w, cin)
+    if w_phase is None or w_phase is False:
+        s.w_phase = None
+        return Call(lib.msd_conv_gemm, (C.byref(s),), name, keep=s)
+    s.w_phase = _p(w_phase)
+    return Call(lib.msd_conv_gemm, (C.byref(s),), name, keep=(s, w_phase))
 
 
 def conv_gemm_ln_slots(*, N, tile_n, tile_m=0, ksize=1, act=ACT_NONE) -> int:
diff --git a/minsdtf_amd/packing.py b/minsdtf_amd/packing.py
--- a/minsdtf_amd/packing.py
+++ b/minsdtf_amd/packing.py
@@ -5,7 +5,7 @@
 import numpy as np
 import torch
 
-from .layout import KERAS, VEC, Packed
+from .layout import KERAS, PHASE_TAPS, VEC, Packed
 
 
 def _dev_bf16(t: torch.Tensor, device) -> torch.Tensor:
@@ -18,6 +18,8 @@
         super().__init__(*a, **kw)
         self.chunk_major_keys = set()
         self._fragment = {}
+        self._phase_host = {}
+        self._phase = {}
 
     def layout(self, key: str) -> int:
         return 1 if key in self.chunk_major_keys else 0
@@ -29,6 +31,12 @@
         self[key] = chunk_major(t)
         self.chunk_major_keys.add(key)
 
+
+    def phase_major(self, key: str) -> Optional[torch.Tensor]:
+        t = self._phase.get(key)
+        if t is None and key in self._phase_host:
+            t = self._phase[key] = self._phase_host[key].to(self[key].device)
+        return t
 
     def fragment_major(self, key: str) -> torch.Tensor:
         t = self._fragment.get(key)
@@ -50,6 +58,26 @@
     w = w_nk.reshape(n // 16, 16, k)[:, order, :]
     w = w.reshape(n // 16, 16, k // 64, 2, 4, 8)
     return w.permute(2, 0, 3, 4, 1, 5).contiguous()
+
+
+def phase_fold(w: torch.Tensor) -> torch.Tensor:
+    assert w.dim() == 4 and w.shape[0] == 3 and w.shape[1] == 3, tuple(w.shape)
+    rows = torch.stack([torch.stack([sum(w[ky] for ky in PHASE_TAPS[py][a]) for a in (0, 1)]) for py in (0, 1)])
+    return torch.stack([torch.stack([sum(rows[:, :, kx] for kx in PHASE_TAPS[px][b]) for b in (0, 1)]) for px in (0, 1)]) \
+        .permute(2, 0, 3, 1, 4, 5).contiguous()
+
+
+def phase_major(w: torch.Tensor) -> torch.Tensor:
+    _, _, cin, n = w.shape
+    assert cin % 64 == 0, cin
+    f = phase_fold(w.to(torch.float32)).reshape(4, 4 * cin, n)
+    return f.to(torch.bfloat16).reshape(4, 4 * cin // 64, 64, n).permute(0, 1, 3, 2).contiguous()
+
+
+def phase_major_of_packed(w_cm: torch.Tensor, cin: int) -> torch.Tensor:
+    nkc, n, _ = w_cm.shape
+    assert nkc * 64 == 9 * cin and cin % 64 == 0, (tuple(w_cm.shape), cin)
+    return phase_major(w_cm.permute(0, 2, 1).reshape(3, 3, cin, n))
 
 
 def chunk_major(w_nk: torch.Tensor) -> torch.Tensor:
@@ -191,6 +219,8 @@
                 masters.vec[lncs], masters.vec[lnb] = W[lncs].clone(), W[lnb].clone()
         if e.chunk_major:
             W.to_chunk_major(e.key)
+        if e.phase and not (keep is not None and not e.sources.isdisjoint(keep)):
+            W._phase_host[e.key] = phase_major(torch.from_numpy(np.ascontiguousarray(_weight(named, e.parts[0].layer), dtype=np.float32)))
     for n in keep or ():
         masters.layer[n] = logical(_weight(named, n)).contiguous().to(device)
     return W, masters
@@ -199,7 +229,7 @@
 def save_packed(W: PackedWeights, path: str, meta: dict = None) -> None:
     import os
 
-    blob = {"meta": dict(meta or {}), "chunk_major": sorted(W.chunk_major_keys),
+    blob = {"meta": dict(meta or {}), "chunk_major": sorted(W.chunk_major_keys), "phase": dict(getattr(W, "_phase_host", {})),
             "tensors": {k: (t.detach().cpu() if isinstance(t, torch.Tensor) else t) for k, t in W.items()}}
     tmp = f"{path}.tmp.{os.getpid()}"
     torch.save(blob, tmp)
@@ -212,4 +242,7 @@
         raise ValueError(f"{path}: packed for {blob['meta']}, wanted {dict(meta)}")
     W = PackedWeights({k: (t.to(device) if isinstance(t, torch.Tensor) else t) for k, t in blob["tensors"].items()})
     W.chunk_major_keys = set(blob["chunk_major"])
+    if "phase" not in blob:
+        raise ValueError(f"{path}: packed without phase images (an earlier version of this package wrote it): pack again")
+    W._phase_host = dict(blob["phase"])
     return W
diff --git a/minsdtf_amd/tuning.py b/minsdtf_amd/tuning.py
--- a/minsdtf_amd/tuning.py
+++ b/minsdtf_amd/tuning.py
@@ -43,12 +43,14 @@
     return next(fam for base, fam in ((6000, None), (5000, "big"), (4000, "wreg"), (3000, "rowpanel"), (1000, "halo"), (tile_m, "tile")) if tile_m >= base)
 
 
-def form_of(tile_m: int, tile_n: int, stages: int = 0) -> Form:
+def form_of(tile_m: int, tile_n: int, stages: int = 0, phase: bool = False) -> Form:
     fam, rows, walk = _family(tile_m), tile_m % 1000, 2 if stages >= 20 else 1 if stages >= 10 else 0
     if fam is None:
         raise ValueError(f"tile_m {tile_m} names no kernel form")
     if fam == "big":
         name = f"staged halo 16x16 x{tile_n}" if walk == 2 else f"big {rows}x{tile_n}" + (" chunk-major" if walk else "")
+        if phase and walk == 2:
+            return Form("bigphase", rows, tile_n, stages - 20, True, 0, 0, f"phase 4 x staged halo 16x16 x{tile_n}")
         return Form("bighalo" if walk == 2 else fam, rows, tile_n, stages - 10 * walk, walk > 0, 0, 0, name)
     if fam == "wreg":
         return Form(fam, rows, tile_n, stages, False, (1 if stages % 20 >= 10 else 0) + (2 if walk == 2 else 0), 0, f"wreg {rows}x{tile_n}" + (" 2K/stage" if walk == 2 else ""))
@@ -90,7 +92,7 @@
             if ov.startswith("@"):
                 with open(ov[1:]) as f:
                     ov = f.read()
-            _table.update({k: list(v) + [0.0] for k, v in json.loads(ov).items()})
+            _table.update({k: list(v[:4]) + [0.0] + list(v[4:]) for k, v in json.loads(ov).items()})
         _families = {}
         for key, ent in _table.items():
             b, rest = key.split("x", 1)
@@ -126,6 +128,8 @@
     if ksize == 3 and stride == 1:
         if cx == 0 and not upsample and w_in % 16 == 0 and h_in % 8 == 0 and hw_out >= 256:
             walk = "chunk"
+        elif cx == 0 and upsample and h_in % 16 == 0 and w_in % 16 == 0:
+            walk = "phase"
         elif cx == 0 and upsample and tile16 and h_in * w_in >= 256:
             walk = "chunk"
         elif cx and w_in % 16 == 0 and h_in % 8 == 0 and hw_out >= 256:
@@ -159,7 +163,7 @@
         if M <= 4096 or N < 80:
             return 1128, 64, sk, 0
         return 1128, (80 if (N % 80 == 0 and allow_split) else 64), sk, 93
-    if walk == "chunk":
+    if walk in ("chunk", "phase"):
         wgs16 = batch * (hl // 16) * (wl // 16) * _ceil_div(N, 128) * sk if tile16 else 0
         if upsample:
             if tile16:
@@ -219,6 +223,8 @@
                         ent = [1128, 80 if (N % 80 == 0 and M > 4096) else 64, int(ent[2]), 93 if M > 4096 else 0, 0.0]
                 elif big.chunk_major and not upsample and stride == 1 and w_in % 16 == 0 and h_in % 8 == 0:
                     ent = [1128, 80 if N % 80 == 0 else 64, int(ent[2]), 0, 0.0]
+                elif big.family == "bighalo" and phase_form(h_in, w_in, cin, N, ksize, stride, upsample, allow_split, cx):
+                    pass
                 elif big.chunk_major:
                     ent = [5256, 128, int(ent[2]), 10, 0.0]
                 else:
@@ -234,8 +240,20 @@
     return shape_config(batch, h_in, w_in, cin, N, ksize, stride, upsample, M, nk, allow_split, cx)
 
 
-def numerics_class(ksize: int, tile_m: int, tile_n: int, splitk: int, ln_producer: bool = True, stages: int = 0) -> Tuple[bool, int, int]:
-    f = form_of(tile_m, tile_n, stages)
+def phase_form(h_in, w_in, cin, N, ksize, stride, upsample, allow_split=True, cx=0) -> bool:
+    if not (ksize == 3 and stride == 1 and upsample and not cx and h_in % 16 == 0 and w_in % 16 == 0 and cin % 64 == 0):
+        return False
+    _load()
+    fam = _families.get(shape_key(0, h_in, w_in, cin, N, ksize, stride, upsample, allow_split, cx).split("x", 1)[1])
+    if fam:
+        return all(len(e) > 5 and bool(e[5]) and form_of(int(e[0]), int(e[1]), int(e[3])).family == "bighalo" for e in fam.values())
+    return shape_class(h_in, w_in, cin, N, ksize, stride, upsample, allow_split, cx)[0] == "phase"
+
+
+def numerics_class(ksize: int, tile_m: int, tile_n: int, splitk: int, ln_producer: bool = True, stages: int = 0, phase: bool = False) -> Tuple[bool, int, int]:
+    f = form_of(tile_m, tile_n, stages, phase)
+    if f.family == "bigphase":
+        return ("phase", splitk, 0)
     cols = 64 if f.family == "rowpanel" else 0 if f.family in ("big", "bighalo") and f.chunk_major else tile_n
     return (f.chunk_major, splitk, cols if (ksize == 1 and ln_producer) else 0)
 
```

Result: no change. 10.36 images/s, median of 6 (+0.8%).
